# adamnelsonarcher/BB-OCR

Measured on AMD Instinct MI355X. Metric: book-page images/sec end-to-end (detect+recognize) @1280x960, higher is better.
Workload: dtype fp16

## Files before the change

### bb-ocr_amd/csrc/abi.cpp

```cpp
#include "ctx.h"

static hipError_t create_seq_stream(hipStream_t* s) {
    return hipStreamCreateWithFlags(s, hipStreamNonBlocking);
}

extern "C" {

void bbocr_default_params(bbocr_params* p) {
    if (!p) return;
    memset(p, 0, sizeof(*p));
    p->text_threshold = 0.7; p->low_text = 0.4; p->link_threshold = 0.4; p->canvas_size = 2560; p->mag_ratio = 1.0;
    p->slope_ths = 0.1; p->ycenter_ths = 0.5; p->height_ths = 0.5; p->width_ths = 0.5; p->add_margin = 0.1; p->min_size = 20;
    p->contrast_ths = 0.1; p->adjust_contrast = 0.5;
    p->decoder = BBOCR_DECODER_GREEDY; p->beam_width = 5;
}

int bbocr_create(const bbocr_config* cfg, bbocr_ctx** out) {
    bbocr_config_v2 v2{};
    if (cfg) v2.base = *cfg;
    return bbocr_create_v2(&v2, out);
}

int bbocr_create_v2(const bbocr_config_v2* cfg, bbocr_ctx** out) {
    if (!out) return BBOCR_ERR_ARG;
    *out = nullptr;
    bbocr_ctx* c = nullptr;
    try {
        c = new bbocr_ctx();
        c->root = c;
        if (cfg) { c->cfg = cfg->base; c->cfg_beam_wide = cfg->beam_wide; }
        if (c->cfg.precision < BBOCR_PREC_BF16 || c->cfg.precision > BBOCR_PREC_EXACT_REC || c->cfg.call_slots < 0 || c->cfg.call_slots > kMaxSlots ||
            c->cfg.rec_quant < 0 || c->cfg.rec_quant > 1 || (c->cfg.rec_quant == 1 && !rec_split(c)) ||
            c->cfg.rec_classes < 0 || rec_classes(c) < 2 || rec_classes(c) > BBOCR_REC_CLASSES_MAX || c->cfg_beam_wide < 0 || c->cfg_beam_wide > 1 ||
            (c->cfg.rec_quant == 1 && rec_classes(c) != kRecClassesDefault)) {
            delete c;
            return BBOCR_ERR_ARG;
        }
        int ndev = 0;
        if (hipGetDeviceCount(&ndev) != hipSuccess || ndev <= 0 || c->cfg.device < 0 || c->cfg.device >= ndev) {
            delete c;
            return BBOCR_ERR_HIP;
        }
        if (hipSetDevice(c->cfg.device) != hipSuccess || hipStreamCreateWithFlags(&c->stream, hipStreamNonBlocking) != hipSuccess ||
            hipStreamCreateWithFlags(&c->stream2, hipStreamNonBlocking) != hipSuccess ||
            create_seq_stream(&c->seq_stream) != hipSuccess ||
            hipMalloc(&c->zero_page, 256) != hipSuccess || hipMemset(c->zero_page, 0, 256) != hipSuccess) {
            delete c;
            return BBOCR_ERR_HIP;
        }
    } catch (...) {
        delete c;
        return BBOCR_ERR_INTERNAL;
    }
    c->cur = c->stream;
    *out = c;
    return BBOCR_OK;
}

}

bbocr_ctx* slot_create(bbocr_ctx* root) {
    bbocr_ctx* s = new bbocr_ctx();
    s->root = root;
    s->cfg = root->cfg;
    s->cfg_beam_wide = root->cfg_beam_wide;
    s->stream = root->stream;
    hipError_t e = hipStreamCreateWithFlags(&s->stream2, hipStreamNonBlocking);
    if (e == hipSuccess) e = create_seq_stream(&s->seq_stream);
    if (e != hipSuccess) {
        if (s->stream2) (void)hipStreamDestroy(s->stream2);
        delete s;
        fail(BBOCR_ERR_HIP, std::string("call slot: ") + hipGetErrorString(e));
    }
    s->cur = s->stream;
    return s;
}

void slot_destroy(bbocr_ctx* c) {
    if (c->stream2) (void)hipStreamSynchronize(c->stream2);
    if (c->seq_stream) (void)hipStreamSynchronize(c->seq_stream);
    if (c->feat_ev) (void)hipEventDestroy(c->feat_ev);
    for (hipEvent_t e : c->sub_events) (void)hipEventDestroy(e);
    if (c->det_t0) { (void)hipEventDestroy(c->det_t0); (void)hipEventDestroy(c->det_t1); }
    if (c->ccl_t0) { (void)hipEventDestroy(c->ccl_t0); (void)hipEventDestroy(c->ccl_t1); }
    if (c->sync_ev) (void)hipEventDestroy(c->sync_ev);
    if (c->seq_t1) { (void)hipEventDestroy(c->seq_t1); (void)hipEventDestroy(c->seq_t2); }
    for (auto& r : c->prof_recs) { (void)hipEventDestroy(r.e0); (void)hipEventDestroy(r.e1); }
    for (hipEvent_t e : c->prof_pool) (void)hipEventDestroy(e);
    DevBuf* bufs[] = {&c->arena.buf, &c->heat, &c->gray, &c->resized, &c->ccl_label, &c->ccl_stat, &c->ccl_slot, &c->ccl_comps, &c->ccl_rowext,
                      &c->ccl_counters, &c->crop_desc, &c->crop_desc2, &c->crop_scratch, &c->crop_hscratch, &c->crop_wscratch, &c->crop_luts, &c->crop_hist,
                      &c->ctc_idx, &c->ctc_pmax, &c->ctc_out_idx, &c->ctc_out, &c->seq_v, &c->seq_xp, &c->seq_h, &c->seq_lin, &c->seq_logits,
                      &c->seq_tables, &c->pp_gray, &c->pp_a, &c->pp_b, &c->pp_c, &c->pp_tab, &c->ctc_probs, &c->ctc_beam_idx, &c->ctc_beam_len, &c->ctc_cand, &c->ctc_cand_n, &c->ac_work, &c->th_coef, &c->je_scan, &c->je_out, &c->pe_out,
                      &c->pg_rgb, &c->pg_tab, &c->seq_q8, &c->seq_rowp, &c->ctc_mask};
    for (DevBuf* b : bufs) b->release();
    if (c->stream2) (void)hipStreamDestroy(c->stream2);
    if (c->seq_stream) (void)hipStreamDestroy(c->seq_stream);
    if (c->root != c) delete c;
}

namespace {
struct ThreadTimes { const bbocr_ctx* root = nullptr; float ms[8] = {0}; int ctc_route = -1; int ctc_host_seqs = 0; };
thread_local ThreadTimes tl_times;
thread_local std::string tl_err;
struct ThreadMask { const bbocr_ctx* root = nullptr; std::vector<unsigned int> words; };
thread_local ThreadMask tl_mask;
}
const unsigned int* thread_class_mask(const bbocr_ctx* root, int* n_words) {
    const bool mine = tl_mask.root == root && !tl_mask.words.empty();
    *n_words = mine ? (int)tl_mask.words.size() : 0;
    return mine ? tl_mask.words.data() : nullptr;
}
void publish_times(const bbocr_ctx* s) {
    tl_times.root = s->root;
    memcpy(tl_times.ms, s->times, sizeof(tl_times.ms));
    tl_times.ctc_route = s->ctc_last_route;
    tl_times.ctc_host_seqs = s->ctc_host_seqs;
}

extern "C" {

void bbocr_destroy(bbocr_ctx* c) {
    if (!c) return;
    if (tl_mask.root == c) tl_mask = ThreadMask();
    if (tl_times.root == c) tl_times = ThreadTimes();
    (void)hipSetDevice(c->cfg.device);
    if (c->stream) (void)hipStreamSynchronize(c->stream);
    dist_release(c);
    for (bbocr_ctx* s : c->slots) slot_destroy(s);
    c->slots.clear();
    free_weights(c);
    slot_destroy(c);
    if (c->zero_page) (void)hipFree(c->zero_page);
    for (SideLane* l : {&c->upload_lane, &c->jpeg_lane})
        if (l->stream) (void)hipStreamDestroy(l->stream);
    if (c->stream) (void)hipStreamDestroy(c->stream);
    delete c;
}

const char* bbocr_last_error(bbocr_ctx* c) {
    if (!c) return "null context";
    std::lock_guard<std::mutex> lk(c->pool_mu);
    tl_err = c->err;
    return tl_err.c_str();
}

int bbocr_load_weights(bbocr_ctx* ctx, int which, const bbocr_tensor_desc* descs, int n) {
    return guarded(ctx, [&](bbocr_ctx* ctx) {
        if (!descs || n <= 0 || (which != 0 && which != 1)) fail(BBOCR_ERR_ARG, "bad weight descriptor table");
        if (which == 0 ? ctx->craft_loaded : ctx->crnn_loaded)
            fail(BBOCR_ERR_STATE, "this network is already loaded: the packed blocks (and the weight blob layout) are fixed per context -- create a new context");
        TensorMap tm(descs, n);
        if (which == 0) load_craft(ctx, tm);
        else load_crnn(ctx, tm);
    }, true);
}

int bbocr_alloc_weights(bbocr_ctx* ctx, int which) {
    return guarded(ctx, [&](bbocr_ctx* ctx) {
        if (which != 0 && which != 1) fail(BBOCR_ERR_ARG, "which: 0 = detector, 1 = recogniser");
        if (which == 0 ? ctx->craft_loaded : ctx->crnn_loaded)
            fail(BBOCR_ERR_STATE, "this network is already laid out in this context -- create a new context");
        TensorMap tm;
        if (which == 0) load_craft(ctx, tm);
        else load_crnn(ctx, tm);
    }, true);
}

int bbocr_weights_blob_size(bbocr_ctx* ctx, size_t* bytes) {
    return guarded(ctx, [&](bbocr_ctx* ctx) {
        if (!bytes) fail(BBOCR_ERR_ARG, "null pointer");
        *bytes = weights_blob_bytes(ctx);
    }, true);
}

int bbocr_weights_export(bbocr_ctx* ctx, void* dev_blob, size_t bytes) {
    return guarded(ctx, [&](bbocr_ctx* ctx) {
        if (!dev_blob) fail(BBOCR_ERR_ARG, "null device pointer");
        weights_export(ctx, dev_blob, bytes);
    }, true);
}

int bbocr_weights_import(bbocr_ctx* ctx, const void* dev_blob, size_t bytes) {
    return guarded(ctx, [&](bbocr_ctx* ctx) {
        if (!dev_blob) fail(BBOCR_ERR_ARG, "null device pointer");
        weights_import(ctx, dev_blob, bytes);
    }, true);
}

int bbocr_detect_dims(int H, int W, int canvas_size, double mag_ratio, int* H32, int* W32, int* rh, int* rw, double* ratio) {
    if (H <= 0 || W <= 0 || canvas_size <= 0) return BBOCR_ERR_ARG;
    const DetDims d = det_dims(H, W, canvas_size, (double)mag_ratio);
    if (H32) *H32 = d.H32;
    if (W32) *W32 = d.W32;
    if (rh) *rh = d.h;
    if (rw) *rw = d.w;
    if (ratio) *ratio = d.ratio;
    return BBOCR_OK;
}

int bbocr_detect(bbocr_ctx* ctx, const uint8_t* dev_rgb, int B, int H, int W, const bbocr_params* p, float* dev_heat_out) {
    return guarded(ctx, [&](bbocr_ctx* ctx) {
        bbocr_params pp;
        bbocr_default_params(&pp);
        if (p) pp = *p;
        if (!dev_rgb || !dev_heat_out) fail(BBOCR_ERR_ARG, "null device pointer");
        memset(ctx->times, 0, sizeof(ctx->times));
        auto t0 = clk::now();
        detect_impl(ctx, dev_rgb, B, H, W, pp, dev_heat_out);
        slot_sync(ctx, ctx->stream);
        prof_collect(ctx);
        ctx->times[0] = ctx->times[7] = (float)ms_since(t0);
    });
}

int bbocr_boxes(bbocr_ctx* ctx, const float* dev_heat, int B, int h, int w, double ratio, const bbocr_params* p, bbocr_boxlist** out) {
    return guarded(ctx, [&](bbocr_ctx* ctx) {
        bbocr_params pp;
        bbocr_default_params(&pp);
        if (p) pp = *p;
        if (!dev_heat || !out) fail(BBOCR_ERR_ARG, "null pointer");
        memset(ctx->times, 0, sizeof(ctx->times));
        auto t0 = clk::now();
        HostBoxes hb;
        boxes_impl(ctx, dev_heat, B, h, w, ratio, pp, hb, ctx->stream);
        *out = export_boxes(hb);
        ctx->times[7] = (float)ms_since(t0);
    });
}

int bbocr_recognize(bbocr_ctx* ctx, const uint8_t* dev_gray, int B, int H, int W, const bbocr_boxlist* boxes, const bbocr_params* p,
                    bbocr_result** out) {
    return guarded(ctx, [&](bbocr_ctx* ctx) {
        bbocr_params pp;
        bbocr_default_params(&pp);
        if (p) pp = *p;
        if (!dev_gray || !boxes || !out || boxes->n_images != B) fail(BBOCR_ERR_ARG, "bad recognise arguments");
        memset(ctx->times, 0, sizeof(ctx->times));
        auto t0 = clk::now();
        HostBoxes hb;
        import_boxes(boxes, hb);
        std::vector<BoxJob> jobs;
        std::vector<int> off;
        recognize_impl(ctx, GrayPages{dev_gray, H, W}, B, hb, pp, jobs, off);
        prof_collect(ctx);
        *out = export_result(B, jobs, off);
        ctx->times[7] = (float)ms_since(t0);
    });
}

int bbocr_readtext_batch(bbocr_ctx* ctx, const uint8_t* dev_rgb, const uint8_t* dev_gray, int B, int H, int W, const bbocr_params* p,
                         bbocr_result** out) {
    return guarded(ctx, [&](bbocr_ctx* ctx) {
        bbocr_params pp;
        bbocr_default_params(&pp);
        if (p) pp = *p;
        if (!dev_rgb || !out) fail(BBOCR_ERR_ARG, "null pointer");
        memset(ctx->times, 0, sizeof(ctx->times));
        auto t_all = clk::now();
        const DetDims d = det_dims(H, W, pp.canvas_size, pp.mag_ratio);
        ctx->heat.ensure((size_t)B * d.h * d.w * 2 * sizeof(float));
        if (!dev_gray) {
            ctx->gray.ensure((size_t)B * H * W);
            HIPCHK(launch_gray(dev_rgb, (uint8_t*)ctx->gray.p, (size_t)B * H * W, ctx->stream));
            dev_gray = (const uint8_t*)ctx->gray.p;
        }
        std::vector<std::pair<int, int>> subs;
        if (!ctx->det_t0) { HIPCHK(hipEventCreate(&ctx->det_t0)); HIPCHK(hipEventCreate(&ctx->det_t1)); }
        HIPCHK(hipEventRecord(ctx->det_t0, ctx->stream));
        detect_impl(ctx, dev_rgb, B, H, W, pp, (float*)ctx->heat.p, [&](int b0, int nb) {
            if (subs.size() >= ctx->sub_events.size()) {
                hipEvent_t e;
                HIPCHK(hipEventCreateWithFlags(&e, hipEventDisableTiming));
                ctx->sub_events.push_back(e);
            }
            HIPCHK(hipEventRecord(ctx->sub_events[subs.size()], ctx->stream));
            subs.push_back({b0, nb});
        });
        HIPCHK(hipEventRecord(ctx->det_t1, ctx->stream));
        HostBoxes hb;
        hb.polys.resize(B); hb.hori.resize(B); hb.freeb.resize(B);
        RecEarly early;
        for (size_t k = 0; k < subs.size(); ++k) {
            const int b0 = subs[k].first, nb = subs[k].second;
            HIPCHK(hipStreamWaitEvent(ctx->stream2, ctx->sub_events[k], 0));
            HostBoxes part;
            boxes_impl(ctx, (const float*)ctx->heat.p + (size_t)b0 * d.h * d.w * 2, nb, d.h, d.w, d.ratio, pp, part, ctx->stream2);
            for (int i = 0; i < nb; ++i) {
                hb.polys[b0 + i] = std::move(part.polys[i]);
                hb.hori[b0 + i] = std::move(part.hori[i]);
                hb.freeb[b0 + i] = std::move(part.freeb[i]);
            }
            if (subs.size() >= 2 && k + 2 == subs.size() && pp.rotation_info[0] == 0 && ctx->crnn_loaded)
                rec_early_begin(ctx, GrayPages{dev_gray, H, W}, b0 + nb, B, hb, pp, early);
        }
        HIPCHK(hipEventSynchronize(ctx->det_t1));
        float det_ms = 0.f;
        HIPCHK(hipEventElapsedTime(&det_ms, ctx->det_t0, ctx->det_t1));
        ctx->times[0] = det_ms;
        std::vector<BoxJob> jobs;
        std::vector<int> off;
        recognize_impl(ctx, GrayPages{dev_gray, H, W}, B, hb, pp, jobs, off, &early);
        prof_collect(ctx);
        *out = export_result(B, jobs, off);
        ctx->times[7] = (float)ms_since(t_all);
    });
}

void bbocr_preproc_defaults(bbocr_preproc_params* p, int legacy) {
    if (!p) return;
    memset(p, 0, sizeof(*p));
    p->scale = 1.5; p->unsharp_radius = 1.0; p->unsharp_threshold = 3;
    if (legacy) { p->blur_sigma = 5.0; p->contrast = 1.3; p->brightness = 0.0; p->clahe_clip = 2.0; p->unsharp_percent = 20; }
    else        { p->blur_sigma = 3.0; p->contrast = 1.9; p->brightness = 1.2; p->clahe_clip = 2.5; p->unsharp_percent = 30; }
}

int bbocr_preprocess_chain(bbocr_ctx* ctx, const uint8_t* dev_bgr, int H, int W, const bbocr_preproc_params* p, uint8_t* dev_out, int* out_h,
                           int* out_w) {
    return guarded(ctx, [&](bbocr_ctx* ctx) {
        bbocr_preproc_params q;
        bbocr_preproc_defaults(&q, 0);
        if (p) q = *p;
        if (H <= 0 || W <= 0) fail(BBOCR_ERR_ARG, "bad image shape");
        if (q.scale < 0 || q.blur_sigma < 0 || q.contrast < 0 || q.brightness < 0 || q.clahe_clip < 0 || q.unsharp_radius < 0 || q.unsharp_percent < 0)
            fail(BBOCR_ERR_ARG, "negative pre-processing parameter");
        const int dh = q.scale > 0 ? (int)(H * q.scale) : H, dw = q.scale > 0 ? (int)(W * q.scale) : W;
        if (out_h) *out_h = dh;
        if (out_w) *out_w = dw;
        if (!dev_out) return;
        if (!dev_bgr) fail(BBOCR_ERR_ARG, "null device pointer");
        if (dh <= 0 || dw <= 0) fail(BBOCR_ERR_ARG, "image collapses to zero size");
        if (q.clahe_clip > 0 && (dh < 16 || dw < 16)) fail(BBOCR_ERR_ARG, "image too small for the 8x8 CLAHE tile grid");
        preprocess_chain_impl(ctx, dev_bgr, H, W, q, dev_out, dh, dw);
    });
}

int bbocr_preprocess_book_cover(bbocr_ctx* ctx, const uint8_t* dev_bgr, int H, int W, uint8_t* dev_out, int* out_h, int* out_w) {
    bbocr_preproc_params q;
    bbocr_preproc_defaults(&q, 0);
    return bbocr_preprocess_chain(ctx, dev_bgr, H, W, &q, dev_out, out_h, out_w);
}

void bbocr_free_boxlist(bbocr_boxlist* b) {
    if (!b) return;
    free(b->poly_off); free(b->polys); free(b->hori_off); free(b->hori); free(b->free_off); free(b->free_q);
    free(b);
}

void bbocr_free_result(bbocr_result* r) {
    if (!r) return;
    free(r->box_off); free(r->quads); free(r->is_free); free(r->text_off); free(r->text_idx); free(r->conf);
    free(r);
}

int bbocr_set_class_mask(bbocr_ctx* ctx, const uint32_t* words, int n_words) {
    return status_of(ctx, [&] {
        if (!rec_wide(ctx)) fail(BBOCR_ERR_ARG, "bbocr_set_class_mask is for contexts of more than 128 classes; bbocr_params::ignore_mask rules here");
        const int C = rec_classes(ctx), max_words = (C + 31) / 32;
        if (n_words < 0 || n_words > max_words || (n_words > 0 && !words)) fail(BBOCR_ERR_ARG, "class mask: 0 .. " + std::to_string(max_words) + " words");
        if (n_words > 0 && (words[0] & 1u)) fail(BBOCR_ERR_ARG, "the CTC blank (class 0) cannot be ignored");
        if (n_words == max_words && (C & 31) && (words[n_words - 1] >> (C & 31))) fail(BBOCR_ERR_ARG, "class mask: a bit behind the last class is set");
        tl_mask.root = n_words > 0 ? ctx : nullptr;
        tl_mask.words.assign(words, words + n_words);
    });
}

int bbocr_last_ctc_route(bbocr_ctx* ctx, int* route) {
    if (!ctx || !route) return BBOCR_ERR_ARG;
    *route = tl_times.root == ctx ? tl_times.ctc_route : -1;
    return BBOCR_OK;
}

int bbocr_last_ctc_host_sequences(bbocr_ctx* ctx, int* n) {
    if (!ctx || !n) return BBOCR_ERR_ARG;
    *n = tl_times.root == ctx ? tl_times.ctc_host_seqs : 0;
    return BBOCR_OK;
}

int bbocr_set_profiling(bbocr_ctx* ctx, int on) {
    return guarded(ctx, [&](bbocr_ctx* c) {
        c->profiling = on < 0 ? 0 : (on > 2 ? 2 : on);
        std::lock_guard<std::mutex> lk(c->pool_mu);
        for (int g = 0; g < 2; ++g) { c->prof_ms[g] = 0; c->prof_flops[g] = 0; c->prof_launches[g] = 0; }
    }, true);
}

int bbocr_conv_profile(bbocr_ctx* ctx, int group, double* ms, double* flops, long long* launches) {
    if (!ctx || group < 0 || group > 1) return BBOCR_ERR_ARG;
    std::lock_guard<std::mutex> lk(ctx->pool_mu);
    if (ms) *ms = ctx->prof_ms[group];
    if (flops) *flops = ctx->prof_flops[group];
    if (launches) *launches = ctx->prof_launches[group];
    return BBOCR_OK;
}

int bbocr_stage_times(bbocr_ctx* ctx, float* ms, int n) {
    if (!ctx || !ms || n <= 0) return BBOCR_ERR_ARG;
    for (int i = 0; i < n && i < 8; ++i) ms[i] = tl_times.root == ctx ? tl_times.ms[i] : 0.f;
    return BBOCR_OK;
}


}
```

### bb-ocr_amd/csrc/ccl.hip

```cpp
#include "common.h"
#include "kernels.h"

__device__ __forceinline__ int ccl_find(const int* __restrict__ label, int x) {
    int p = __hip_atomic_load(label + x, __ATOMIC_RELAXED, __HIP_MEMORY_SCOPE_AGENT);
    while (p != x) {
        x = p;
        p = __hip_atomic_load(label + x, __ATOMIC_RELAXED, __HIP_MEMORY_SCOPE_AGENT);
    }
    return x;
}

__device__ __forceinline__ void ccl_union(int* label, int a, int b) {
    for (;;) {
        a = ccl_find(label, a);
        b = ccl_find(label, b);
        if (a == b) return;
        if (a > b) { const int t = a; a = b; b = t; }
        const int old = atomicMin(label + b, a);
        if (old == b) return;
        b = old;
    }
}

__global__ void __launch_bounds__(256) ccl_init_kernel(const float* __restrict__ heat, size_t total, int w, float low_text, float link_thr,
                                                       int* __restrict__ label, int* __restrict__ stat, int* __restrict__ slot) {
    const int lane = threadIdx.x & 63;
    const size_t nround = (total + (size_t)gridDim.x * 256 - 1) / ((size_t)gridDim.x * 256);
    for (size_t it = 0; it < nround; ++it) {
        const size_t i = (it * gridDim.x + blockIdx.x) * 256 + threadIdx.x;
        bool fg = false;
        int x = 0;
        if (i < total) {
            const float2 v = *(const float2*)(heat + i * 2);
            fg = (v.x > low_text) || (v.y > link_thr);
            x = (int)(i % w);
        }
        const unsigned long long fgm = __ballot(fg);
        const bool start = fg && (lane == 0 || x == 0 || !((fgm >> (lane - 1)) & 1ULL));
        const unsigned long long sm = __ballot(start);
        if (i < total) {
            int lab = -1;
            if (fg) {
                const unsigned long long below = sm & ((lane == 63) ? ~0ULL : ((1ULL << (lane + 1)) - 1ULL));
                lab = (int)i - (lane - (63 - __clzll((long long)below)));
            }
            label[i] = lab;
            slot[i] = -1;
            int* st = stat + i * 6;
            st[0] = 0x7fffffff; st[1] = -1; st[2] = 0x7fffffff; st[3] = -1; st[4] = 0; st[5] = 0;
        }
    }
}

__global__ void __launch_bounds__(256) ccl_merge_kernel(size_t total, int h, int w, int* label) {
    for (size_t i = (size_t)blockIdx.x * 256 + threadIdx.x; i < total; i += (size_t)gridDim.x * 256) {
        if (label[i] < 0) continue;
        const int x = (int)(i % w);
        const int y = (int)((i / w) % h);
        const bool left = x > 0 && label[i - 1] >= 0;
        if (left && (i & 63) == 0) ccl_union(label, (int)i, (int)i - 1);
        if (y > 0 && label[i - w] >= 0 && !(left && label[i - w - 1] >= 0)) ccl_union(label, (int)i, (int)i - w);
    }
}

__global__ void __launch_bounds__(256) ccl_stats_kernel(const float* __restrict__ heat, size_t total, int h, int w, int* label,
                                                        int* __restrict__ stat) {
    const int lane = threadIdx.x & 63;
    const size_t nround = (total + (size_t)gridDim.x * 256 - 1) / ((size_t)gridDim.x * 256);
    for (size_t it = 0; it < nround; ++it) {
        const size_t i = (it * gridDim.x + blockIdx.x) * 256 + threadIdx.x;
        int r = -1, x = 0, y = 0;
        float t = 0.f;
        if (i < total && label[i] >= 0) {
            r = ccl_find(label, (int)i);
            label[i] = r;
            x = (int)(i % w);
            y = (int)((i / w) % h);
            t = fmaxf(heat[i * 2], 0.f);
        }
        const int rp = __shfl_up(r, 1);
        const bool head = r >= 0 && (lane == 0 || rp != r || x == 0);
        const unsigned long long hm = __ballot(head || r < 0);
        if (r >= 0) {
            const unsigned long long below = hm & ((lane == 63) ? ~0ULL : ((1ULL << (lane + 1)) - 1ULL));
            const int first = 63 - __clzll((long long)below);
            const unsigned long long above = (lane == 63) ? 0ULL : (hm >> (lane + 1));
            const int len_after = above ? (__ffsll((long long)above) - 1) : (63 - lane);
            float m = t;
#pragma unroll
            for (int o = 1; o < 64; o <<= 1) {
                const float mo = __shfl_down(m, o);
                if (o <= len_after) m = fmaxf(m, mo);
            }
            if (head) {
                int* st = stat + (size_t)r * 6;
                atomicMin(st + 0, x);
                atomicMax(st + 1, x + len_after);
                atomicMin(st + 2, y);
                atomicMax(st + 3, y);
                atomicAdd(st + 4, len_after + 1);
                if (m > 0.f) atomicMax(st + 5, __float_as_int(m));
            }
            (void)first;
        }
    }
}

__global__ void __launch_bounds__(256) ccl_accept_kernel(size_t total, int hw, double text_thr, const int* __restrict__ label,
                                                         const int* __restrict__ stat, int* __restrict__ slot, CclOut* comps,
                                                         int* rowext, int* counters, int cap_comps, int cap_rows) {
    for (size_t i = (size_t)blockIdx.x * 256 + threadIdx.x; i < total; i += (size_t)gridDim.x * 256) {
        if (label[i] != (int)i) continue;
        const int* st = stat + i * 6;
        const int area = st[4];
        if (area < 10) continue;
        if ((double)__int_as_float(st[5]) < text_thr) continue;
        const int img = (int)(i / hw);
        const int hh = st[3] - st[2] + 1;
        const int idx = atomicAdd(counters + 0, 1);
        const int off = atomicAdd(counters + 1, hh);
        if (idx >= cap_comps || off + hh > cap_rows) { atomicOr(counters + 2, 1); continue; }
        CclOut c;
        c.root = (int)(i - (size_t)img * hw);
        c.left = st[0]; c.top = st[2]; c.right = st[1]; c.bottom = st[3]; c.area = area; c.row_off = off; c.img = img;
        comps[idx] = c;
        slot[i] = idx;
        int* re = rowext + (size_t)off * 2;
        for (int k = 0; k < hh; ++k) { re[2 * k] = 0x7fffffff; re[2 * k + 1] = -1; }
    }
}

__global__ void __launch_bounds__(256) ccl_rowext_kernel(const float* __restrict__ heat, size_t total, int h, int w, float low_text,
                                                         const int* __restrict__ label, const int* __restrict__ slot,
                                                         const CclOut* __restrict__ comps, int* rowext, int cap_comps, int cap_rows) {
    const int lane = threadIdx.x & 63;
    const size_t nround = (total + (size_t)gridDim.x * 256 - 1) / ((size_t)gridDim.x * 256);
    for (size_t it = 0; it < nround; ++it) {
        const size_t i = (it * gridDim.x + blockIdx.x) * 256 + threadIdx.x;
        int r = -1, x = 0;
        if (i < total) {
            r = label[i];
            if (r >= 0 && !(heat[i * 2] > low_text)) r = -1;
            x = (int)(i % w);
        }
        const int rp = __shfl_up(r, 1);
        const bool head = r >= 0 && (lane == 0 || rp != r || x == 0);
        const unsigned long long hm = __ballot(head || r < 0);
        if (head) {
            const int s = slot[r];
            if (s >= 0) {
                const unsigned long long above = (lane == 63) ? 0ULL : (hm >> (lane + 1));
                const int len_after = above ? (__ffsll((long long)above) - 1) : (63 - lane);
                const CclOut c = comps[s];
                const int y = (int)((i / w) % h);
                int* re = rowext + ((size_t)c.row_off + (y - c.top)) * 2;
                atomicMin(re, x);
                atomicMax(re + 1, x + len_after);
            }
        }
    }
}

hipError_t launch_ccl(const float* heat, int N, int h, int w, float low_text, float link_thr, double text_thr, int* label, int* stat,
                      int* slot, CclOut* comps, int* rowext, int* counters, int cap_comps, int cap_rows, hipStream_t s) {
    const size_t total = (size_t)N * h * w;
    if (total == 0) return hipSuccess;
    if (total > 0x7fffffffULL) return hipErrorInvalidValue;
    const int grid = (int)((total + 255) / 256 < 16384 ? (total + 255) / 256 : 16384);
    hipError_t e = hipMemsetAsync(counters, 0, sizeof(int) * 4, s);
    if (e != hipSuccess) return e;
    hipLaunchKernelGGL(ccl_init_kernel, dim3(grid), dim3(256), 0, s, heat, total, w, low_text, link_thr, label, stat, slot);
    hipLaunchKernelGGL(ccl_merge_kernel, dim3(grid), dim3(256), 0, s, total, h, w, label);
    hipLaunchKernelGGL(ccl_stats_kernel, dim3(grid), dim3(256), 0, s, heat, total, h, w, label, stat);
    hipLaunchKernelGGL(ccl_accept_kernel, dim3(grid), dim3(256), 0, s, total, h * w, text_thr, label, stat, slot, comps, rowext, counters,
                       cap_comps, cap_rows);
    hipLaunchKernelGGL(ccl_rowext_kernel, dim3(grid), dim3(256), 0, s, heat, total, h, w, low_text, label, slot, comps, rowext, cap_comps,
                       cap_rows);
    return hipGetLastError();
}
```

### bb-ocr_amd/csrc/crnn_misc.hip

```cpp
#include "common.h"
#include "kernels.h"

template <bool PAGES>
__global__ void __launch_bounds__(256) crop_warp_kernel(const uint8_t* __restrict__ gray, int H, int W, const CropDesc* __restrict__ descs,
                                                        int first, uint8_t* __restrict__ wscratch, const CropPage* __restrict__ pages) {
    const CropDesc d = descs[first + blockIdx.y];
    if (!d.warp) return;
    const uint8_t* src;
    size_t pitch;
    if constexpr (PAGES) {
        const CropPage pg = pages[d.img];
        src = gray + pg.off; H = pg.H; W = pg.W; pitch = (size_t)pg.pitch;
    } else {
        src = gray + (size_t)d.img * H * W; pitch = (size_t)W;
    }
    uint8_t* dst = wscratch + d.warp_off;
    const int total = d.sw * d.sh;
    for (int i = blockIdx.x * 256 + threadIdx.x; i < total; i += gridDim.x * 256) {
        const int x = i % d.sw, y = i / d.sw;
        const double X0 = d.Minv[0] * (double)x + (d.Minv[1] * (double)y + d.Minv[2]);
        const double Y0 = d.Minv[3] * (double)x + (d.Minv[4] * (double)y + d.Minv[5]);
        const double W0 = d.Minv[6] * (double)x + (d.Minv[7] * (double)y + d.Minv[8]);
        const double Wi = W0 != 0.0 ? 32.0 / W0 : 0.0;
        double fX = X0 * Wi, fY = Y0 * Wi;
        fX = fX < -2147483648.0 ? -2147483648.0 : (fX > 2147483647.0 ? 2147483647.0 : fX);
        fY = fY < -2147483648.0 ? -2147483648.0 : (fY > 2147483647.0 ? 2147483647.0 : fY);
        const long long X = (long long)rint(fX), Y = (long long)rint(fY);
        long long sxl = X >> 5, syl = Y >> 5;
        sxl = sxl < -32768 ? -32768 : (sxl > 32767 ? 32767 : sxl);
        syl = syl < -32768 ? -32768 : (syl > 32767 ? 32767 : syl);
        const int sx = (int)sxl, sy = (int)syl;
        const int ax = (int)(X & 31), ay = (int)(Y & 31);
        auto tap = [&](int yy, int xx) -> int {
            return (yy >= 0 && yy < H && xx >= 0 && xx < W) ? (int)src[(size_t)yy * pitch + xx] : 0;
        };
        const int acc = tap(sy, sx) * ((32 - ax) * (32 - ay) * 32) + tap(sy, sx + 1) * (ax * (32 - ay) * 32) +
                        tap(sy + 1, sx) * ((32 - ax) * ay * 32) + tap(sy + 1, sx + 1) * (ax * ay * 32);
        int v = (acc + (1 << 14)) >> 15;
        dst[i] = (uint8_t)(v < 0 ? 0 : (v > 255 ? 255 : v));
    }
}

__device__ __forceinline__ void cv_lin_coef_d(int d, int ssize, double scale, int& s0, int& s1, int& a0, int& a1) {
    float fx = (float)(((double)d + 0.5) * scale - 0.5);
    int sx = (int)floorf(fx);
    fx -= (float)sx;
    if (sx < 0) { fx = 0.f; sx = 0; }
    if (sx >= ssize - 1) { fx = 0.f; sx = ssize - 1; }
    a0 = __float2int_rn((1.f - fx) * 2048.f);
    a1 = __float2int_rn(fx * 2048.f);
    s0 = sx;
    s1 = sx + 1 < ssize ? sx + 1 : ssize - 1;
}

template <bool PAGES>
__global__ void __launch_bounds__(256) crop_resize_kernel(const uint8_t* __restrict__ gray, int H, int W, const CropDesc* __restrict__ descs,
                                                          int first, const uint8_t* __restrict__ wscratch, uint8_t* __restrict__ scratch,
                                                          const CropPage* __restrict__ pages) {
    const CropDesc d = descs[first + blockIdx.y];
    const uint8_t* src;
    size_t stride;
    if (d.warp) { src = wscratch + d.warp_off; stride = (size_t)d.sw; }
    else if constexpr (PAGES) {
        const CropPage pg = pages[d.img];
        src = gray + pg.off + (size_t)d.sy0 * (size_t)pg.pitch + d.sx0; stride = (size_t)pg.pitch;
    }
    else { src = gray + (size_t)d.img * H * W + (size_t)d.sy0 * W + d.sx0; stride = (size_t)W; }
    uint8_t* dst = scratch + d.a_off;
    const int sw = d.sw, sh = d.sh, dw = (d.rot & 1) ? d.rh : d.rw, dh = (d.rot & 1) ? d.rw : d.rh;
    const bool same = (dw == sw && dh == sh), area2 = (sw == 2 * dw && sh == 2 * dh);
    const double scale_x = 1.0 / ((double)dw / (double)sw), scale_y = 1.0 / ((double)dh / (double)sh);
    const int total = dw * dh;
    for (int i = blockIdx.x * 256 + threadIdx.x; i < total; i += gridDim.x * 256) {
        const int dx = i % dw, dy = i / dw;
        int v;
        if (same) {
            v = src[(size_t)dy * stride + dx];
        } else if (area2) {
            v = (src[(size_t)(2 * dy) * stride + 2 * dx] + src[(size_t)(2 * dy) * stride + 2 * dx + 1] +
                 src[(size_t)(2 * dy + 1) * stride + 2 * dx] + src[(size_t)(2 * dy + 1) * stride + 2 * dx + 1] + 2) >> 2;
        } else {
            int x0, x1, a0, a1, y0, y1, b0, b1;
            cv_lin_coef_d(dx, sw, scale_x, x0, x1, a0, a1);
            cv_lin_coef_d(dy, sh, scale_y, y0, y1, b0, b1);
            const int r0 = src[(size_t)y0 * stride + x0] * a0 + src[(size_t)y0 * stride + x1] * a1;
            const int r1 = src[(size_t)y1 * stride + x0] * a0 + src[(size_t)y1 * stride + x1] * a1;
            v = (((b0 * (r0 >> 4)) >> 16) + ((b1 * (r1 >> 4)) >> 16) + 2) >> 2;
            v = v < 0 ? 0 : (v > 255 ? 255 : v);
        }
        int o = i;
        if (d.rot == 1) o = (dw - 1 - dx) * dh + dy;
        else if (d.rot == 2) o = (dh - 1 - dy) * dw + (dw - 1 - dx);
        else if (d.rot == 3) o = dx * dh + (dh - 1 - dy);
        dst[o] = (uint8_t)v;
    }
}

__global__ void __launch_bounds__(256) crop_hist_kernel(const uint8_t* __restrict__ scratch, const CropDesc* __restrict__ descs, int first,
                                                        unsigned int* __restrict__ hist) {
    __shared__ unsigned int h[256];
    const CropDesc d = descs[first + blockIdx.x];
    h[threadIdx.x] = 0;
    __syncthreads();
    const uint8_t* p = scratch + d.a_off;
    const int total = d.rw * d.rh;
    for (int i = threadIdx.x; i < total; i += 256) atomicAdd(&h[p[i]], 1u);
    __syncthreads();
    hist[(size_t)blockIdx.x * 256 + threadIdx.x] = h[threadIdx.x];
}

#define PIL_PREC 22
__device__ __forceinline__ double pil_bicubic(double x) {
    const double a = -0.5;
    if (x < 0.0) x = -x;
    if (x < 1.0) return ((a + 2.0) * x - (a + 3.0)) * x * x + 1;
    if (x < 2.0) return (((x - 5) * x + 8) * x - 4) * a;
    return 0.0;
}
struct PilWin { int x0, n; double center, ss, ww; };
__device__ PilWin pil_window(int in_size, int out_size, int xx) {
    double scale = (double)in_size / (double)out_size, filterscale = scale;
    if (filterscale < 1.0) filterscale = 1.0;
    const double support = 2.0 * filterscale;
    PilWin w;
    w.center = ((double)xx + 0.5) * scale;
    w.ss = 1.0 / filterscale;
    int x0 = (int)(w.center - support + 0.5);
    if (x0 < 0) x0 = 0;
    int x1 = (int)(w.center + support + 0.5);
    if (x1 > in_size) x1 = in_size;
    w.x0 = x0;
    w.n = x1 - x0;
    w.ww = 0.0;
    for (int x = 0; x < w.n; ++x) w.ww += pil_bicubic(((double)(x + x0) - w.center + 0.5) * w.ss);
    return w;
}
__device__ __forceinline__ int pil_tap(const PilWin& w, int x) {
    double k = pil_bicubic(((double)(x + w.x0) - w.center + 0.5) * w.ss);
    if (w.ww != 0.0) k = k / w.ww;
    return k < 0 ? (int)(-0.5 + k * (double)(1 << PIL_PREC)) : (int)(0.5 + k * (double)(1 << PIL_PREC));
}
__device__ __forceinline__ int pil_clip8(long long v) {
    const long long r = v >> PIL_PREC;
    return r < 0 ? 0 : (r > 255 ? 255 : (int)r);
}

__global__ void __launch_bounds__(256) crop_pil_h_kernel(const CropDesc* __restrict__ descs, int first, const uint8_t* __restrict__ scratch,
                                                         const uint8_t* __restrict__ luts, uint8_t* __restrict__ hscratch) {
    const CropDesc d = descs[first + blockIdx.y];
    if (d.fw == d.rw && d.rh == 64) return;
    const uint8_t* src = scratch + d.a_off;
    const uint8_t* lut = d.lut_off >= 0 ? luts + d.lut_off : nullptr;
    uint8_t* dst = hscratch + d.a_off;
    const int total = d.rh * d.fw;
    for (int i = blockIdx.x * 256 + threadIdx.x; i < total; i += gridDim.x * 256) {
        const int xx = i % d.fw, y = i / d.fw;
        int v;
        if (d.fw == d.rw) {
            v = src[(size_t)y * d.rw + xx];
            if (lut) v = lut[v];
        } else {
            const PilWin win = pil_window(d.rw, d.fw, xx);
            long long acc = 1LL << (PIL_PREC - 1);
            for (int k = 0; k < win.n; ++k) {
                int p = src[(size_t)y * d.rw + win.x0 + k];
                if (lut) p = lut[p];
                acc += (long long)p * pil_tap(win, k);
            }
            v = pil_clip8(acc);
        }
        dst[i] = (uint8_t)v;
    }
}

template <int MODE>
__global__ void __launch_bounds__(256) crop_final_kernel(const CropDesc* __restrict__ descs, int first, const uint8_t* __restrict__ scratch,
                                                         const uint8_t* __restrict__ hscratch, const uint8_t* __restrict__ luts,
                                                         uint16_t* __restrict__ out, int row_stride, long long slot_stride, int gap) {
    const CropDesc d = descs[first + blockIdx.y];
    const bool tall = !(d.fw == d.rw && d.rh == 64);
    const uint8_t* src = (tall ? hscratch : scratch) + d.a_off;
    const uint8_t* lut = (!tall && d.lut_off >= 0) ? luts + d.lut_off : nullptr;
    uint16_t* dst = out + (size_t)d.slot * (size_t)slot_stride;
    const int imgW = d.imgW;
    const int t = blockIdx.x * 256 + threadIdx.x;
    const int y = t >> 6, x0 = t & 63;
    if (y >= 64) return;
    const bool vert = tall && d.rh != 64;
    PilWin win;
    if (vert) win = pil_window(d.rh, 64, y);
    auto sample = [&](int xs) {
        int v;
        if (!tall) {
            v = src[(size_t)y * d.rw + xs];
            if (lut) v = lut[v];
        } else if (!vert) {
            v = src[(size_t)y * d.fw + xs];
        } else {
            long long acc = 1LL << (PIL_PREC - 1);
            for (int k = 0; k < win.n; ++k) acc += (long long)src[(size_t)(win.x0 + k) * d.fw + xs] * pil_tap(win, k);
            v = pil_clip8(acc);
        }
        if constexpr (MODE == REC_SPLIT) return (unsigned short)(v + 1);
        else return El<MODE == REC_F16 ? 1 : 0>::from_f32(((float)v / 255.0f - 0.5f) / 0.5f);
    };
    uint16_t* drow = dst + (size_t)y * row_stride;
    for (int x = imgW + x0; x < imgW + gap; x += 64) drow[x] = 0;
    int x = x0;
    for (; x < d.fw; x += 64) drow[x] = sample(x);
    if (x < imgW) {
        const uint16_t edge = sample(d.fw - 1);
        for (; x < imgW; x += 64) drow[x] = edge;
    }
}

hipError_t launch_crops(const uint8_t* gray, int H, int W, const CropDesc* descs_dev, int first, int count, int imgW, int any_warp,
                        int any_tall, uint8_t* wscratch, uint8_t* scratch, uint8_t* hscratch, const uint8_t* luts, uint16_t* out_bucket,
                        int stage_mask, hipStream_t s, int wide_row_stride, int gap, int mode, const CropPage* pages) {
    if (count <= 0) return hipSuccess;
    if ((stage_mask & 1) && pages) {
        if (any_warp) hipLaunchKernelGGL(crop_warp_kernel<true>, dim3(16, count), dim3(256), 0, s, gray, 0, 0, descs_dev, first, wscratch, pages);
        hipLaunchKernelGGL(crop_resize_kernel<true>, dim3(16, count), dim3(256), 0, s, gray, 0, 0, descs_dev, first, wscratch, scratch, pages);
    } else if (stage_mask & 1) {
        if (any_warp) hipLaunchKernelGGL(crop_warp_kernel<false>, dim3(16, count), dim3(256), 0, s, gray, H, W, descs_dev, first, wscratch, pages);
        hipLaunchKernelGGL(crop_resize_kernel<false>, dim3(16, count), dim3(256), 0, s, gray, H, W, descs_dev, first, wscratch, scratch, pages);
    }
    if (stage_mask & 2) {
        if (any_tall) hipLaunchKernelGGL(crop_pil_h_kernel, dim3(8, count), dim3(256), 0, s, descs_dev, first, scratch, luts, hscratch);
        const int rs = wide_row_stride > 0 ? wide_row_stride : imgW;
        const long long ss = wide_row_stride > 0 ? 1LL : (long long)64 * imgW;
        const int gp = wide_row_stride > 0 ? gap : 0;
        if (mode == REC_SPLIT)
            hipLaunchKernelGGL(crop_final_kernel<REC_SPLIT>, dim3(16, count), dim3(256), 0, s, descs_dev, first, scratch, hscratch, luts, out_bucket, rs, ss, gp);
        else if (mode == REC_F16)
            hipLaunchKernelGGL(crop_final_kernel<REC_F16>, dim3(16, count), dim3(256), 0, s, descs_dev, first, scratch, hscratch, luts, out_bucket, rs, ss, gp);
        else
            hipLaunchKernelGGL(crop_final_kernel<REC_BF16>, dim3(16, count), dim3(256), 0, s, descs_dev, first, scratch, hscratch, luts, out_bucket, rs, ss, gp);
    }
    return hipGetLastError();
}

hipError_t launch_crop_hist(const uint8_t* scratch, const CropDesc* descs_dev, int first, int count, unsigned int* hist, hipStream_t s) {
    if (count <= 0) return hipSuccess;
    hipLaunchKernelGGL(crop_hist_kernel, dim3(count), dim3(256), 0, s, scratch, descs_dev, first, hist);
    return hipGetLastError();
}

template <int MODE>
__global__ void __launch_bounds__(256) crnn_conv0_kernel(const uint16_t* __restrict__ in, const float* __restrict__ w,
                                                         const float* __restrict__ b, uint16_t* __restrict__ out, int n, int W) {
    const int OW = W / 2, OH = 32;
    const size_t total = (size_t)n * OH * OW;
    for (size_t i = (size_t)blockIdx.x * 256 + threadIdx.x; i < total; i += (size_t)gridDim.x * 256) {
        const int ox = (int)(i % OW);
        const size_t r = i / OW;
        const int oy = (int)(r % OH);
        const int img = (int)(r / OH);
        const uint16_t* p = in + (size_t)img * 64 * W;
        float v[4][4];
#pragma unroll
        for (int dy = 0; dy < 4; ++dy)
#pragma unroll
            for (int dx = 0; dx < 4; ++dx) {
                const int iy = 2 * oy - 1 + dy, ix = 2 * ox - 1 + dx;
                float x = 0.f;
                if (iy >= 0 && iy < 64 && ix >= 0 && ix < W) {
                    const unsigned short q = p[(size_t)iy * W + ix];
                    if constexpr (MODE == REC_SPLIT) x = q ? ((float)(q - 1) / 255.0f - 0.5f) / 0.5f : 0.f;
                    else x = El<MODE == REC_F16 ? 1 : 0>::to_f32(q);
                }
                v[dy][dx] = x;
            }
        uint16_t* op = out + i * (MODE == REC_SPLIT ? 64 : 32);
#pragma unroll 1
        for (int c8 = 0; c8 < 32; c8 += 8) {
            u32x4 o, ol;
#pragma unroll
            for (int c2 = 0; c2 < 4; ++c2) {
                const int c = c8 + c2 * 2;
                const f32x2_t bias = {b[c], b[c + 1]};
                f32x2_t best = {0.f, 0.f};
#pragma unroll
                for (int py = 0; py < 2; ++py)
#pragma unroll
                    for (int px = 0; px < 2; ++px) {
                        f32x2_t a = bias;
#pragma unroll
                        for (int ky = 0; ky < 3; ++ky)
#pragma unroll
                            for (int kx = 0; kx < 3; ++kx) {
                                const f32x2_t wv = *(const f32x2_t*)(w + (ky * 3 + kx) * 32 + c);
                                const float x = v[py + ky][px + kx];
                                a = __builtin_elementwise_fma(wv, (f32x2_t){x, x}, a);
                            }
                        best = __builtin_elementwise_max(best, a);
                    }
                if constexpr (MODE == REC_SPLIT) {
                    const float h0 = El<1>::to_f32(El<1>::from_f32(best[0])), h1 = El<1>::to_f32(El<1>::from_f32(best[1]));
                    o[c2] = El<1>::pack2(h0, h1);
                    ol[c2] = El<1>::pack2((best[0] - h0) * SPLIT_LO_SCALE, (best[1] - h1) * SPLIT_LO_SCALE);
                } else {
                    o[c2] = El<MODE == REC_F16 ? 1 : 0>::pack2(best[0], best[1]);
                }
            }
            *(u32x4*)(op + c8) = o;
            if constexpr (MODE == REC_SPLIT) *(u32x4*)(op + 32 + c8) = ol;
        }
    }
}

void pack_crnn_conv0_mfma(const float* w_tap_major, uint16_t* out, int el) {
    size_t o = 0;
    for (int j = 0; j < 2; ++j)
        for (int l = 0; l < 64; ++l) {
            const int m = l & 15, kg = l >> 4;
            const int cout = 8 * (m >> 2) + 4 * j + (m & 3);
            for (int t = 0; t < 8; ++t) {
                const float v = w_tap_major[t * 32 + cout];
                const float hi = el_to_f32_host(el, f32_to_el_host(el, v));
                const float lo = el_to_f32_host(el, f32_to_el_host(el, v - hi));
                const float lo2 = el_to_f32_host(el, f32_to_el_host(el, (v - hi) - lo));
                out[o++] = f32_to_el_host(el, kg == 0 ? hi : (kg == 1 ? lo : (kg == 2 ? lo2 : 0.f)));
            }
        }
}

template <int EL>
__global__ void __launch_bounds__(256) crnn_conv0_mfma_kernel(const uint16_t* __restrict__ in, const uint16_t* __restrict__ afrag, const float* __restrict__ w,
                                                              const float* __restrict__ b, uint16_t* __restrict__ out, int W) {
    constexpr int TW = 64, PITCH = TW + 16, ROWS = 66;
    __shared__ __attribute__((aligned(16))) uint16_t tile[ROWS * PITCH];
    typedef typename El<EL>::v8 v8;
    const int tid = threadIdx.x, lane = tid & 63, wave = tid >> 6;
    const int g = lane >> 4, n = lane & 15;
    const int x0 = blockIdx.x * TW, img = blockIdx.y;
    const int OW = W >> 1;
    const uint16_t* src = in + (size_t)img * 64 * W;
    for (int idx = tid; idx < ROWS * (PITCH / 4); idx += 256) {
        const int row = idx / (PITCH / 4), ch = idx - row * (PITCH / 4);
        const int iy = row - 1, ix = x0 - 8 + ch * 4;
        u32x2 v = {0u, 0u};
        if (iy >= 0 && iy < 64 && ix >= 0 && ix + 4 <= W) v = *(const u32x2*)(src + (size_t)iy * W + ix);
        *(u32x2*)(tile + row * PITCH + ch * 4) = v;
    }
    const v8 a0 = *(const v8*)(afrag + (size_t)lane * 8), a1 = *(const v8*)(afrag + (size_t)(64 + lane) * 8);
    float w8[8], bi[8];
#pragma unroll
    for (int i = 0; i < 8; ++i) {
        w8[i] = w[8 * 32 + 8 * g + i];
        bi[i] = b[8 * g + i];
    }
    __syncthreads();
    auto frag = [&](int y, int cf, f32x4& d0, f32x4& d1) {
        const uint16_t* p = tile + (y + 1) * PITCH + 8 + cf * 16 + n;
        u32x4 bq;
#pragma unroll
        for (int i = 0; i < 4; ++i) {
            const int t0 = 2 * i, t1 = 2 * i + 1;
            const unsigned int lo = p[(t0 / 3 - 1) * PITCH + (t0 % 3 - 1)], hi = p[(t1 / 3 - 1) * PITCH + (t1 % 3 - 1)];
            bq[i] = lo | (hi << 16);
        }
        const float x8 = El<EL>::to_f32(p[PITCH + 1]);
        d0 = El<EL>::mfma(a0, __builtin_bit_cast(v8, bq), (f32x4){bi[0], bi[1], bi[2], bi[3]});
        d1 = El<EL>::mfma(a1, __builtin_bit_cast(v8, bq), (f32x4){bi[4], bi[5], bi[6], bi[7]});
#pragma unroll
        for (int r = 0; r < 4; ++r) {
            d0[r] = fmaf(w8[r], x8, d0[r]);
            d1[r] = fmaf(w8[4 + r], x8, d1[r]);
        }
    };
#pragma unroll 1
    for (int rp = 0; rp < 8; ++rp) {
        const int y = 2 * (wave * 8 + rp);
#pragma unroll
        for (int cf = 0; cf < 4; ++cf) {
            f32x4 u0, u1, l0, l1;
            frag(y, cf, u0, u1);
            frag(y + 1, cf, l0, l1);
            float m[8];
#pragma unroll
            for (int r = 0; r < 4; ++r) {
                m[r] = __builtin_fmaxf(__builtin_fmaxf(u0[r], l0[r]), 0.f);
                m[4 + r] = __builtin_fmaxf(__builtin_fmaxf(u1[r], l1[r]), 0.f);
            }
#pragma unroll
            for (int i = 0; i < 8; ++i)
                m[i] = fmaxf(m[i], __int_as_float(__builtin_amdgcn_update_dpp(0, __float_as_int(m[i]), 0xB1 , 0xF, 0xF, true)));
            const int px = (x0 + cf * 16 + n) >> 1;
            if (!(n & 1) && px < OW) {
                const u32x4 o = {El<EL>::pack2(m[0], m[1]), El<EL>::pack2(m[2], m[3]), El<EL>::pack2(m[4], m[5]), El<EL>::pack2(m[6], m[7])};
                *(u32x4*)(out + (((size_t)img * 32 + (y >> 1)) * OW + px) * 32 + 8 * g) = o;
            }
        }
    }
}

hipError_t launch_crnn_conv0(const uint16_t* in, const float* w, const float* b, uint16_t* out, int n, int W, int mode, hipStream_t s,
                             const uint16_t* afrag) {
    const size_t total = (size_t)n * 32 * (W / 2);
    if (total == 0) return hipSuccess;
    if (afrag && mode != REC_SPLIT && (W & 3) == 0 && n <= 65535) {
        const dim3 grid((W + 63) / 64, n);
        if (mode == REC_F16) hipLaunchKernelGGL(crnn_conv0_mfma_kernel<1>, grid, dim3(256), 0, s, in, afrag, w, b, out, W);
        else hipLaunchKernelGGL(crnn_conv0_mfma_kernel<0>, grid, dim3(256), 0, s, in, afrag, w, b, out, W);
        return hipGetLastError();
    }
    const int grid = (int)((total + 255) / 256 < 16384 ? (total + 255) / 256 : 16384);
    if (mode == REC_SPLIT) hipLaunchKernelGGL(crnn_conv0_kernel<REC_SPLIT>, dim3(grid), dim3(256), 0, s, in, w, b, out, n, W);
    else if (mode == REC_F16) hipLaunchKernelGGL(crnn_conv0_kernel<REC_F16>, dim3(grid), dim3(256), 0, s, in, w, b, out, n, W);
    else hipLaunchKernelGGL(crnn_conv0_kernel<REC_BF16>, dim3(grid), dim3(256), 0, s, in, w, b, out, n, W);
    return hipGetLastError();
}

template <int MODE>
__device__ __forceinline__ void rowmean3_8(const uint16_t* p0, const uint16_t* p1, const uint16_t* p2, uint16_t* o, int lo_off) {
    typedef El<MODE == REC_BF16 ? 0 : 1> E;
    const u32x4 a = *(const u32x4*)(p0), bq = *(const u32x4*)(p1), c = *(const u32x4*)(p2);
    u32x4 oh, ol;
    if constexpr (MODE == REC_SPLIT) {
        const u32x4 al = *(const u32x4*)(p0 + lo_off), bl = *(const u32x4*)(p1 + lo_off), cl = *(const u32x4*)(p2 + lo_off);
        const float inv = 1.0f / SPLIT_LO_SCALE;
#pragma unroll
        for (int j = 0; j < 4; ++j) {
            const f32x2_t m = ((E::unpack2(a[j]) + E::unpack2(al[j]) * inv) + (E::unpack2(bq[j]) + E::unpack2(bl[j]) * inv) +
                               (E::unpack2(c[j]) + E::unpack2(cl[j]) * inv)) / 3.0f;
            const f32x2_t h = E::unpack2(E::pack2(m[0], m[1]));
            oh[j] = E::pack2(h[0], h[1]);
            ol[j] = E::pack2((m[0] - h[0]) * SPLIT_LO_SCALE, (m[1] - h[1]) * SPLIT_LO_SCALE);
        }
        *(u32x4*)(o) = oh;
        *(u32x4*)(o + lo_off) = ol;
    } else {
#pragma unroll
        for (int j = 0; j < 4; ++j) {
            const f32x2_t m = (E::unpack2(a[j]) + E::unpack2(bq[j]) + E::unpack2(c[j])) / 3.0f;
            oh[j] = E::pack2(m[0], m[1]);
        }
        *(u32x4*)(o) = oh;
    }
}

__global__ void __launch_bounds__(256) crnn_zero_gaps_kernel(uint16_t* __restrict__ t, const CropDesc* __restrict__ descs, int first, int H, int Wl,
                                                             int C8, int shift, int gapw) {
    const CropDesc d = descs[first + blockIdx.x];
    const int x0 = (d.slot + d.imgW) >> shift;
    const int total = H * gapw * C8;
    for (int i = threadIdx.x; i < total; i += 256) {
        const int c8 = i % C8, r = i / C8;
        const int gx = r % gapw, y = r / gapw;
        if (x0 + gx < Wl) *(u32x4*)(t + ((size_t)y * Wl + x0 + gx) * C8 * 8 + (size_t)c8 * 8) = (u32x4){0u, 0u, 0u, 0u};
    }
}
hipError_t launch_crnn_zero_gaps(uint16_t* t, const CropDesc* descs_dev, int first, int count, int H, int Wl, int C, int shift, hipStream_t s) {
    if (count <= 0) return hipSuccess;
    hipLaunchKernelGGL(crnn_zero_gaps_kernel, dim3(count), dim3(256), 0, s, t, descs_dev, first, H, Wl, C / 8, shift, 4 >> shift);
    return hipGetLastError();
}

template <int MODE>
__global__ void __launch_bounds__(256) rowmean3_gather_kernel(const uint16_t* __restrict__ in, int Wc, int C8, const CropDesc* __restrict__ descs,
                                                              int first, uint16_t* __restrict__ out) {
    constexpr int M = MODE == REC_SPLIT ? 2 : 1;
    const CropDesc d = descs[first + blockIdx.y];
    const int T = d.imgW / 4 - 1, xs = d.slot >> 2;
    const size_t plane = (size_t)Wc * C8 * 8 * M;
    const int total = T * C8;
    for (int i = blockIdx.x * 256 + threadIdx.x; i < total; i += gridDim.x * 256) {
        const int t = i / C8, c8 = i - t * C8;
        const uint16_t* p = in + ((size_t)(xs + t) * C8 * M + c8) * 8;
        rowmean3_8<MODE>(p, p + plane, p + 2 * plane, out + ((size_t)(d.pad_ + t) * C8 * M + c8) * 8, C8 * 8);
    }
}
hipError_t launch_rowmean3_gather(const uint16_t* in, int Wc, int C, const CropDesc* descs_dev, int first, int count, uint16_t* out, int mode,
                                  hipStream_t s) {
    if (count <= 0) return hipSuccess;
    if (mode == REC_SPLIT) hipLaunchKernelGGL(rowmean3_gather_kernel<REC_SPLIT>, dim3(8, count), dim3(256), 0, s, in, Wc, C / 8, descs_dev, first, out);
    else if (mode == REC_F16) hipLaunchKernelGGL(rowmean3_gather_kernel<REC_F16>, dim3(8, count), dim3(256), 0, s, in, Wc, C / 8, descs_dev, first, out);
    else hipLaunchKernelGGL(rowmean3_gather_kernel<REC_BF16>, dim3(8, count), dim3(256), 0, s, in, Wc, C / 8, descs_dev, first, out);
    return hipGetLastError();
}
```

### bb-ocr_amd/csrc/ctx.h

```cpp
#pragma once
#include "../../include/bbocr.h"

#include <algorithm>
#include <atomic>
#include <chrono>
#include <condition_variable>
#include <cmath>
#include <cstring>
#include <functional>
#include <map>
#include <memory>
#include <mutex>
#include <string>
#include <thread>
#include <unordered_map>
#include <vector>

#include "boxpost.h"
#include "hostpool.h"
#include "common.h"
#include "kernels.h"


using clk = std::chrono::steady_clock;
static inline double ms_since(clk::time_point t0) { return std::chrono::duration<double, std::milli>(clk::now() - t0).count(); }
static inline size_t align_up(size_t v, size_t a) { return (v + a - 1) / a * a; }
static inline int cdiv(int a, int b) { return (a + b - 1) / b; }

struct StatusError {
    int code;
    std::string msg;
};
[[noreturn]] inline void fail(int code, const std::string& m) { throw StatusError{code, m}; }
#define HIPCHK(expr)                                                                                   \
    do {                                                                                               \
        hipError_t _e = (expr);                                                                        \
        if (_e != hipSuccess) fail(BBOCR_ERR_HIP, std::string(#expr) + ": " + hipGetErrorString(_e));  \
    } while (0)

struct DevBuf {
    void* p = nullptr;
    size_t cap = 0;
    DevBuf() = default;
    DevBuf(const DevBuf&) = delete;
    DevBuf& operator=(const DevBuf&) = delete;
    ~DevBuf() { release(); }
    void ensure(size_t n) {
        if (n <= cap) return;
        if (p) (void)hipFree(p);
        p = nullptr;
        cap = 0;
        HIPCHK(hipMalloc(&p, n));
        cap = n;
    }
    void ensure_keep(size_t n, size_t used) {
        if (n <= cap) return;
        void* q = nullptr;
        HIPCHK(hipDeviceSynchronize());
        HIPCHK(hipMalloc(&q, n));
        if (p && used) HIPCHK(hipMemcpy(q, p, std::min(used, cap), hipMemcpyDeviceToDevice));
        if (p) (void)hipFree(p);
        p = q;
        cap = n;
    }
    void release() {
        if (p) (void)hipFree(p);
        p = nullptr;
        cap = 0;
    }
};

struct PinBuf {
    void* p = nullptr;
    size_t cap = 0;
    PinBuf() = default;
    PinBuf(const PinBuf&) = delete;
    PinBuf& operator=(const PinBuf&) = delete;
    ~PinBuf() { if (p) (void)hipHostFree(p); }
    void ensure(size_t n) {
        if (n <= cap) return;
        if (p) { HIPCHK(hipDeviceSynchronize()); (void)hipHostFree(p); }
        p = nullptr;
        cap = 0;
        HIPCHK(hipHostMalloc(&p, n, hipHostMallocDefault));
        cap = n;
    }
};

struct Arena {
    DevBuf buf;
    size_t off = 0;
    bool dry = true;
    void begin(bool d) { off = 0; dry = d; }
    template <typename T> T* alloc(size_t count) {
        off = align_up(off, 256);
        T* r = dry ? nullptr : (T*)((char*)buf.p + off);
        off += count * sizeof(T);
        return r;
    }
};

struct Carve {
    size_t off = 0;
    size_t add(size_t bytes) { const size_t o = off; off = align_up(off + bytes, 256); return o; }
    template <typename T> static T* at(void* base, size_t o) { return (T*)((char*)base + o); }
};

struct Act {
    uint16_t* p;
    int N, H, W, C;
};

struct DevPage {
    const void* p;
    int H, W;
    long long pitch;
    int layout;
};
constexpr unsigned page_set(int layout) { return 1u << layout; }
constexpr unsigned PAGE_ANY = page_set(PAGE_YCC3 + 1) - 1;
inline void check_page(const DevPage& g, unsigned allowed = PAGE_ANY) {
    if (!g.p) fail(BBOCR_ERR_ARG, "null device pointer");
    if (g.H < 1 || g.W < 1) fail(BBOCR_ERR_ARG, "bad image shape");
    if ((long long)g.H * g.W >= (1LL << 30)) fail(BBOCR_ERR_ARG, "image too large");
    if (g.layout < PAGE_GRAY || g.layout > PAGE_YCC3 || !(allowed & page_set(g.layout))) fail(BBOCR_ERR_ARG, "layout must be one of the BBOCR_PAGE_* taken here");
    if (g.pitch < (long long)g.W * page_px_bytes(g.layout)) fail(BBOCR_ERR_ARG, "row pitch smaller than a row");
}

struct SideLane {
    std::mutex mu;
    hipStream_t stream = nullptr;
};



struct WeightView {
    bool craft_loaded = false;
    uint16_t* c11_wf = nullptr;
    float* c11_b = nullptr;
    float* c11_w32 = nullptr;
    float* cls6_w32 = nullptr;
    ConvPlan conv1_2, conv2_1, conv2_2, conv3_1, conv3_2, conv3_3, conv4_1, conv4_2, conv4_3, conv5_1, conv5_2, fc6, fc7;
    ConvPlan up1a, up1b, up2b, up3b, up4b, cls0, cls2, cls4;
    ConvPlan up2y, up2s, up3y, up3s, up4y, up4s;
    float* cls_tail = nullptr;
    uint16_t* cls_tail_frag = nullptr;
    uint16_t* up4y_post = nullptr;
    bool crnn_loaded = false;
    float* r0_wb = nullptr;
    uint16_t* r0_afrag = nullptr;
    ConvPlan r1, r2, r3, r4, r5, r6, xproj[2], lin[2], pred;
    uint16_t* pred_wide = nullptr;
    float* pred_wide_b = nullptr;
    uint16_t* whh[2] = {nullptr, nullptr};
    float whh_scale[2] = {1.f, 1.f};
    struct Q8Layer { int8_t* w = nullptr; float* scale = nullptr; float* bias = nullptr; };
    Q8Layer q_ih[2], q_hh[2], q_lin[2], q_pred;
    void* zero_page = nullptr;
};

struct bbocr_ctx : WeightView {
    bbocr_config cfg{};
    int cfg_beam_wide = 0;
    bbocr_ctx* root = nullptr;
    std::vector<bbocr_ctx*> slots;
    std::mutex pool_mu;
    std::condition_variable pool_cv;
    std::mutex enq_mu;
    ConvRoute op_conv_route{};
    bool slot_busy = false;
    hipStream_t stream = nullptr;
    DevBuf pp_gray, pp_a, pp_b, pp_c, pp_tab;
    DevBuf ac_work;
    DevBuf th_coef;
    int th_coef_key[6] = {0, 0, 0, 0, 0, 0};
    int th_coef_ks[2] = {0, 0};
    int th_coef_rows[2] = {0, 0};
    DevBuf je_scan, je_out;
    DevBuf pe_out;
    DevBuf pp_cubic;
    int pp_cubic_key[4] = {0, 0, 0, 0};
    unsigned long long pp_cubic_K[2] = {0, 0};
    unsigned int ignore_mask[4] = {0, 0, 0, 0};
    int beam_width = 0;
    std::vector<unsigned int> class_mask;
    DevBuf ctc_mask;
    int ctc_host_seqs = 0;
    int ctc_last_route = -1;
    hipStream_t cur = nullptr;
    SideLane upload_lane;
    SideLane jpeg_lane;
    PinBuf jd_pin;
    DevBuf jd_in, jd_work, jd_coef, jd_stage;
    DevBuf jd_page;
    long long jd_count[4] = {0, 0, 0, 0};
    hipStream_t seq_stream = nullptr;
    hipEvent_t feat_ev = nullptr;
    hipStream_t stream2 = nullptr;
    std::vector<hipEvent_t> sub_events;
    hipEvent_t ccl_t0 = nullptr, ccl_t1 = nullptr;
    hipEvent_t det_t0 = nullptr, det_t1 = nullptr;
    hipEvent_t sync_ev = nullptr;
    hipEvent_t seq_t1 = nullptr, seq_t2 = nullptr;
    std::string err;
    float times[8] = {0};

    struct ProfRec { hipEvent_t e0, e1; double flops; int group; };
    int profiling = 0;
    int prof_group = 0;
    std::vector<ProfRec> prof_recs;
    std::vector<hipEvent_t> prof_pool;
    double prof_ms[2] = {0, 0}, prof_flops[2] = {0, 0};
    long long prof_launches[2] = {0, 0};

    void* dist_comm = nullptr;
    int dist_rank = 0, dist_world = 0;
    std::unique_ptr<HostPool> pool;
    std::vector<void*> owned;
    std::vector<size_t> owned_bytes;

    Arena arena;
    DevBuf heat, gray, resized;
    DevBuf pg_rgb, pg_tab;
    PinBuf pg_pin;
    DevBuf ccl_label, ccl_stat, ccl_slot, ccl_comps, ccl_rowext, ccl_counters;
    DevBuf crop_desc, crop_scratch, crop_hscratch, crop_wscratch, crop_luts, crop_hist;
    DevBuf ctc_idx, ctc_pmax, ctc_out_idx, ctc_out, ctc_probs, ctc_beam_idx, ctc_beam_len, ctc_cand, ctc_cand_n, crop_desc2;
    PinBuf desc_pin, desc_pin2;
    PinBuf ctc_pin;
    DevBuf seq_v, seq_xp, seq_h, seq_lin, seq_logits, seq_tables;
    DevBuf seq_q8, seq_rowp;
};

inline int det_el(const bbocr_ctx* c) { return (c->cfg.precision == BBOCR_PREC_FP16 || c->cfg.precision == BBOCR_PREC_EXACT || c->cfg.precision == BBOCR_PREC_EXACT_REC) ? 1 : 0; }
inline int rec_el(const bbocr_ctx* c) { return c->cfg.precision != BBOCR_PREC_BF16 ? 1 : 0; }
inline bool rec_split(const bbocr_ctx* c) { return c->cfg.precision == BBOCR_PREC_EXACT || c->cfg.precision == BBOCR_PREC_EXACT_REC; }
inline bool rec_quant(const bbocr_ctx* c) { return c->cfg.rec_quant == 1; }
constexpr int kRecClassesDefault = 97;
inline int rec_classes(const bbocr_ctx* c) { return c->cfg.rec_classes > 0 ? c->cfg.rec_classes : kRecClassesDefault; }
inline int rec_cs(const bbocr_ctx* c) { return (rec_classes(c) + 15) / 16 * 16; }
inline bool rec_wide(const bbocr_ctx* c) { return rec_classes(c) > 128; }
inline bool rec_beam_wide(const bbocr_ctx* c) { return c->cfg_beam_wide == 1 && rec_wide(c); }
inline bool det_split(const bbocr_ctx* c) { return c->cfg.precision == BBOCR_PREC_EXACT; }

struct TensorMap {
    std::unordered_map<std::string, const bbocr_tensor_desc*> m;
    bool zeros = false;
    std::vector<float> zero_buf;
    TensorMap() : zeros(true), zero_buf((size_t)5 << 20, 0.f) {}
    TensorMap(const bbocr_tensor_desc* d, int n) {
        for (int i = 0; i < n; ++i) {
            std::string k = d[i].name ? d[i].name : "";
            if (k.rfind("module.", 0) == 0) k = k.substr(7);
            m[k] = &d[i];
        }
    }
    const float* get(const std::string& name, size_t numel, bool required = true) const {
        if (zeros) {
            if (zero_buf.size() < numel) fail(BBOCR_ERR_INTERNAL, "allocation-only load: tensor '" + name + "' larger than the zero buffer");
            return zero_buf.data();
        }
        auto it = m.find(name);
        if (it == m.end()) {
            if (required) fail(BBOCR_ERR_WEIGHTS, "missing tensor '" + name + "'");
            return nullptr;
        }
        size_t n = 1;
        for (int i = 0; i < it->second->ndim; ++i) n *= (size_t)it->second->shape[i];
        if (n != numel || !it->second->data)
            fail(BBOCR_ERR_WEIGHTS, "tensor '" + name + "' has " + std::to_string(n) + " elements, expected " + std::to_string(numel));
        return it->second->data;
    }
};

struct RgbSource { const uint8_t* rgb; int Himg, Wimg; };

struct DetDims {
    int H32, W32, h, w, th, tw;
    double ratio;
};

struct DetPlan {
    int H, W;
    DetDims d;
    std::vector<int> passes;
    size_t arena_bytes, resized_bytes;
};

struct GrayPages {
    const uint8_t* gray;
    int H, W;
    const CropPage* tab = nullptr;
    const CropPage* tab_dev = nullptr;
    int h(int b) const { return tab ? tab[b].H : H; }
    int w(int b) const { return tab ? tab[b].W : W; }
};

struct HostBoxes {
    std::vector<std::vector<std::array<int, 8>>> polys;
    std::vector<std::vector<std::array<int, 4>>> hori;
    std::vector<std::vector<std::array<double, 8>>> freeb;
};

struct BoxJob {
    int img;
    bool is_free;
    double quad[8];
    CropDesc d;
    std::vector<int> text;
    double conf = 0.0;
};

struct RecChunk {
    int imgW, T, first, n;
    size_t row0;
};

struct RecPart {
    std::vector<CropDesc> descs;
    std::vector<int> order;
    std::vector<RecChunk> chunks;
    size_t rows = 0, cols = 0;
    bool any_warp = false, any_tall = false;
};

struct RecRun {
    std::vector<int> tiles, seqs, seq_k;
    size_t rows = 0;
    int n_results = 0;
};

struct RecEarly {
    bool active = false;
    int pages = 0;
    std::vector<BoxJob> jobs;
    std::vector<int> box_off;
    size_t a_total = 0, w_total = 0;
    RecPart part;
};

constexpr int REC_GAP = 4;
constexpr int REC_STAGES = 8;

template <typename T> inline T* upload(bbocr_ctx* c, const std::vector<T>& v) {
    void* d = nullptr;
    HIPCHK(hipMalloc(&d, v.size() * sizeof(T)));
    c->owned.push_back(d);
    c->owned_bytes.push_back(v.size() * sizeof(T));
    HIPCHK(hipMemcpy(d, v.data(), v.size() * sizeof(T), hipMemcpyHostToDevice));
    return (T*)d;
}

ConvPlan make_plan(int Cin, int Cout, int KH, int KW, int pad, int dil, int el = 0, int bn = 0);
void upload_plan(bbocr_ctx* c, ConvPlan& p, const std::vector<float>& w, const std::vector<float>& b);
void free_weights(bbocr_ctx* c);
size_t weights_blob_bytes(const bbocr_ctx* c);
void weights_export(bbocr_ctx* c, void* dev_dst, size_t bytes);
void weights_import(bbocr_ctx* c, const void* dev_src, size_t bytes);
void load_craft(bbocr_ctx* c, const TensorMap& tm);
void load_crnn(bbocr_ctx* c, const TensorMap& tm);
ConvArgs conv_args(const ConvPlan& p, const Act& a0, const Act* a1 = nullptr, const Act* addup = nullptr);
hipError_t launch_conv_profiled(bbocr_ctx* c, const ConvPlan& p, ConvArgs a, bool may_decline = false);
void run_conv(bbocr_ctx* c, const ConvPlan& p, const Act& a0, bool relu0, const Act* a1, bool relu1, bool relu_out, void* out, int out_cs, int cout_store, bool out_f32, const Act* addup = nullptr);
hipError_t launch_seq_proj_profiled(bbocr_ctx* c, const ConvPlan& p, const uint16_t* x, size_t rows_pad, uint16_t* out);
void prof_collect(bbocr_ctx* c);
Act conv_act(bbocr_ctx* c, const ConvPlan& p, const Act& a0, bool relu0, const Act* a1, bool relu1, bool relu_out, int store);
Act conv_pool_act(bbocr_ctx* c, const ConvPlan& p, const Act& a0, bool relu0, bool relu_out, int store, int mode, bool pool_relu, Act* full, const RgbSource* rgb = nullptr);
Act pool_act(bbocr_ctx* c, const Act& a, int kh, int kw, int sh, int sw, int ph, int pw, bool relu_in);
void craft_up_stage(bbocr_ctx* c, const ConvPlan& py, const ConvPlan& ps, const Act& y, const Act& skip, uint16_t* z, uint16_t* out);
bool craft_up3b_post(bbocr_ctx* c, const Act& u3a, uint16_t* u3b, uint16_t* z);
bool craft_up4(bbocr_ctx* c, const Act& s1, const uint16_t* z, uint16_t* u4b);
void craft_cls_tail(bbocr_ctx* c, const Act& c2, float* heat);
struct ExactConvRow {
    const char* name;
    ConvPlan bbocr_ctx::* plan;
    bool relu_out;
    int store;
    int pool_mode;
    bool pool_relu;
    bool keep_full;
};
int craft_exact_rows();
const ExactConvRow& craft_exact_row(int row);
Act craft_exact_conv(bbocr_ctx* c, int row, const Act& in, Act* full = nullptr);
Act craft_exact_conv1_1(bbocr_ctx* c, const uint8_t* rgb, int nb, int Himg, int Wimg, int H32, int W32);
Act craft_exact_relu(bbocr_ctx* c, const Act& a);
Act craft_exact_upcat(bbocr_ctx* c, const Act& y, const Act& skip);
Act craft_exact_pool5(bbocr_ctx* c, const Act& s4);
void craft_exact_cls_tail(bbocr_ctx* c, const Act& c3, float* heat);
DetDims det_dims(int H, int W, int canvas, double mag);
void detect_impl(bbocr_ctx* c, const uint8_t* rgb, int B, int H, int W, const bbocr_params& p, float* heat, const std::function<void(int, int)>& after_sub = nullptr);
DetPlan det_plan(bbocr_ctx* c, int B, int H, int W, const bbocr_params& p, bool overlapped);
void det_size(bbocr_ctx* c, size_t arena_bytes, size_t resized_bytes);
void det_run(bbocr_ctx* c, const DetPlan& s, const uint8_t* rgb, float* heat, const std::function<void(int, int)>& after_sub = nullptr);
int ccl_cap_comps(int B, int h, int w);
void ccl_size(bbocr_ctx* c, size_t npx, int cap_comps);
void boxes_impl(bbocr_ctx* c, const float* heat, int B, int h, int w, double ratio, const bbocr_params& p, HostBoxes& hb, hipStream_t st);
bbocr_boxlist* export_boxes(const HostBoxes& hb);
void import_boxes(const bbocr_boxlist* bl, HostBoxes& hb);
bool plan_horizontal(const std::array<int, 4>& box, int img, int H, int W, BoxJob& j);
bool plan_free(const std::array<double, 8>& fq, int img, BoxJob& j);
int rec_mode(const bbocr_ctx* c);
void crop_refit_fw(CropDesc& d);
void rec_layout_scratch(std::vector<BoxJob>& jobs, size_t first, size_t& a_total, size_t& w_total);
bool contrast_lut(const unsigned int* hist, size_t npx, double target, uint8_t* lut);
std::vector<int> crop_contrast_luts(bbocr_ctx* c, const CropDesc* descs_dev, std::vector<CropDesc>& descs, double target, std::vector<uint8_t>& luts);
void rec_launch_crops(bbocr_ctx* c, const GrayPages& g, const RecPart& part, const CropDesc* dd, uint16_t* wide, int stage);
void rec_plan_part(const std::vector<BoxJob>& jobs, const std::vector<int>& sel, int res0, size_t row_base, RecPart& part);
const CropDesc* rec_upload_descs(bbocr_ctx* c, const RecPart& part, DevBuf& desc_buf);
uint16_t* rec_wide_image(bbocr_ctx* c, const RecPart& part);
void crnn_features_wide(bbocr_ctx* c, const RecPart& part, const CropDesc* descs, const uint16_t* wide);
Act crnn_stage_shape(const bbocr_ctx* c, const RecPart& part, int stage);
Act crnn_features_stages(bbocr_ctx* c, const RecPart& part, const CropDesc* descs, Act a, int first, int last);
void rec_add_tables(RecRun& run, const RecPart& part, int tile_seqs);
void crnn_sequence(bbocr_ctx* c, size_t rows, size_t rows_pad, const int* tiles_dev, int ntiles, const int* seqs_dev, int nseq, float* logits);
void crnn_seq_xproj(bbocr_ctx* c, int l, const uint16_t* x, size_t rows_pad, void* xp);
void crnn_seq_xproj_conv(bbocr_ctx* c, int l, const uint16_t* x, size_t rows_pad, void* xp);
void crnn_seq_lin(bbocr_ctx* c, int l, const uint16_t* h, size_t rows_pad, uint16_t* out);
void crnn_seq_pred(bbocr_ctx* c, const uint16_t* x, size_t rows_pad, float* logits);
void rec_seq_tiles(const bbocr_ctx* c, RecRun& run);
enum { CTC_GREEDY = 0, CTC_BEAM_HOST = 1, CTC_BEAM_DEVICE = 2, CTC_GREEDY_FUSED = 3, CTC_BEAM_DEVICE_WIDE = 4 };
int ctc_route(int beam_width, int C, const int* seqs, int nseq, bool fused_ok = false, bool beam_wide = false);
int ctc_beam_wide_fallback(bbocr_ctx* c, hipStream_t s, const float* probs_dev, const int* seqs, int nseq, int C, int cs, int beam_width, const int* blen,
                           std::vector<std::vector<int>>& texts);
const unsigned int* thread_class_mask(const bbocr_ctx* root, int* n_words);
void ctc_size(bbocr_ctx* c, size_t rows, int nseq, int cs, int route);
double ctc_decode(const CtcOut& o, const int* idx, int n, std::vector<int>& text);
void rec_early_begin(bbocr_ctx* c, const GrayPages& g, int pages, int B, const HostBoxes& hb, const bbocr_params& p, RecEarly& e);
void recognize_impl(bbocr_ctx* c, const GrayPages& g, int B, const HostBoxes& hb, const bbocr_params& p, std::vector<BoxJob>& jobs, std::vector<int>& box_off, RecEarly* early = nullptr);
bbocr_result* export_result(int B, const std::vector<BoxJob>& jobs, const std::vector<int>& box_off);
void pp_resize(bbocr_ctx* c, const uint8_t* src, int H, int W, uint8_t* dst, int dh, int dw, bool src_bgr = false);
void pp_gauss(bbocr_ctx* c, const uint8_t* src, int H, int W, uint8_t* dst, double sigma);
const uint8_t* pp_fold_lut(bbocr_ctx* c, size_t n, double contrast, double brightness);
void pp_clahe(bbocr_ctx* c, const uint8_t* src, int H, int W, const uint8_t* d_lut, uint8_t* dst, double clip_limit);
void pp_unsharp(bbocr_ctx* c, const uint8_t* src, int H, int W, uint8_t* dst, uint8_t* tmp1, uint8_t* tmp2, float radius, int percent, int threshold);
void preprocess_chain_impl(bbocr_ctx* c, const uint8_t* bgr, int H, int W, const bbocr_preproc_params& q, uint8_t* out, int dh, int dw);
void gaussian_taps_fixed(int n, double sigma, int* k);

inline HostPool& host_pool(bbocr_ctx* c) {
    if (!c->pool) {
        const int want = c->cfg.host_threads > 0 ? c->cfg.host_threads : std::min(16, host_cpu_share());
        c->pool.reset(new HostPool(std::max(1, std::min(want, 64)) - 1));
    }
    return *c->pool;
}

inline bool other_call_in_flight(bbocr_ctx* c) {
    bbocr_ctx* root = c->root;
    std::lock_guard<std::mutex> lk(root->pool_mu);
    if (root != c && root->slot_busy) return true;
    for (bbocr_ctx* s : root->slots)
        if (s != c && s->slot_busy) return true;
    return false;
}

struct EnqLock {
    std::unique_lock<std::mutex> lk;
    explicit EnqLock(bbocr_ctx* c) : lk(c->root->enq_mu) {}
};
constexpr int kMaxSlots = 2;
bbocr_ctx* slot_create(bbocr_ctx* root);
void slot_destroy(bbocr_ctx* s);
void publish_times(const bbocr_ctx* s);
void dist_release(bbocr_ctx* root);

inline void slot_sync(bbocr_ctx* c, hipStream_t st) {
    if (!c->sync_ev) HIPCHK(hipEventCreateWithFlags(&c->sync_ev, hipEventDisableTiming));
    HIPCHK(hipEventRecord(c->sync_ev, st));
    HIPCHK(hipEventSynchronize(c->sync_ev));
}

inline void prof_release(bbocr_ctx* c, const bbocr_ctx::ProfRec& r) { c->prof_pool.push_back(r.e0); c->prof_pool.push_back(r.e1); }

inline void guarded_drain(bbocr_ctx* ctx) {
    if (ctx->stream) (void)hipStreamSynchronize(ctx->stream);
    if (ctx->stream2) (void)hipStreamSynchronize(ctx->stream2);
    if (ctx->seq_stream) (void)hipStreamSynchronize(ctx->seq_stream);
    ctx->cur = ctx->stream;
    (void)hipGetLastError();
    for (auto& r : ctx->prof_recs) prof_release(ctx, r);
    ctx->prof_recs.clear();
}

struct SlotLease {
    bbocr_ctx* root;
    bbocr_ctx* slot = nullptr;
    bool exclusive;
    SlotLease(bbocr_ctx* r, bool excl) : root(r), exclusive(excl) {
        std::unique_lock<std::mutex> lk(root->pool_mu);
        const int max_slots = root->cfg.call_slots == 1 ? 1 : kMaxSlots;
        if (exclusive) {
            root->pool_cv.wait(lk, [&] {
                if (root->slot_busy) return false;
                for (bbocr_ctx* s : root->slots) if (s->slot_busy) return false;
                return true;
            });
            root->slot_busy = true;
            for (bbocr_ctx* s : root->slots) s->slot_busy = true;
            slot = root;
            return;
        }
        for (;;) {
            if (!root->slot_busy) { slot = root; break; }
            for (bbocr_ctx* s : root->slots) if (!s->slot_busy) { slot = s; break; }
            if (slot) break;
            if ((int)root->slots.size() + 1 < max_slots) {
                slot = slot_create(root);
                root->slots.push_back(slot);
                break;
            }
            root->pool_cv.wait(lk);
        }
        slot->slot_busy = true;
        if (slot != root) {
            static_cast<WeightView&>(*slot) = static_cast<const WeightView&>(*root);
            slot->cfg = root->cfg;
            slot->cfg_beam_wide = root->cfg_beam_wide;
            slot->profiling = root->profiling;
        }
    }
    ~SlotLease() {
        {
            std::lock_guard<std::mutex> lk(root->pool_mu);
            if (exclusive) {
                root->slot_busy = false;
                for (bbocr_ctx* s : root->slots) s->slot_busy = false;
            } else if (slot) {
                slot->slot_busy = false;
            }
        }
        root->pool_cv.notify_all();
    }
};

inline void set_err(bbocr_ctx* root, const std::string& m) {
    std::lock_guard<std::mutex> lk(root->pool_mu);
    root->err = m;
}

template <typename F> inline int status_of(bbocr_ctx* root, F&& f) {
    if (!root) return BBOCR_ERR_ARG;
    try {
        f();
        return BBOCR_OK;
    } catch (const StatusError& se) {
        set_err(root, se.msg);
        return se.code;
    } catch (const std::exception& ex) {
        set_err(root, ex.what());
        return BBOCR_ERR_INTERNAL;
    } catch (...) {
        set_err(root, "unknown failure");
        return BBOCR_ERR_INTERNAL;
    }
}

template <typename F> inline int guarded(bbocr_ctx* root, F&& f, bool exclusive = false) {
    return status_of(root, [&] {
        HIPCHK(hipSetDevice(root->cfg.device));
        SlotLease lease(root, exclusive);
        bbocr_ctx* ctx = lease.slot;
        try {
            ctx->cur = ctx->stream;
            HIPCHK(hipStreamSynchronize(nullptr));
            f(ctx);
            publish_times(ctx);
        } catch (...) {
            guarded_drain(ctx);
            throw;
        }
    });
}

template <typename F> inline int lane_guarded(bbocr_ctx* root, SideLane bbocr_ctx::*which, bool wait_default, F&& f) {
    return status_of(root, [&] {
        HIPCHK(hipSetDevice(root->cfg.device));
        SideLane& lane = root->*which;
        std::lock_guard<std::mutex> lk(lane.mu);
        try {
            if (!lane.stream) HIPCHK(hipStreamCreateWithFlags(&lane.stream, hipStreamNonBlocking));
            if (wait_default) HIPCHK(hipStreamSynchronize(nullptr));
            f(lane.stream);
        } catch (...) {
            if (lane.stream) (void)hipStreamSynchronize(lane.stream);
            (void)hipGetLastError();
            throw;
        }
    });
}
```

### bb-ocr_amd/csrc/detector.cpp

```cpp
#include "ctx.h"

static hipEvent_t prof_event(bbocr_ctx* c) {
    hipEvent_t e;
    if (!c->prof_pool.empty()) { e = c->prof_pool.back(); c->prof_pool.pop_back(); }
    else HIPCHK(hipEventCreate(&e));
    return e;
}

template <typename F> static hipError_t profiled(bbocr_ctx* c, double flops, F&& launch) {
    if (c->profiling == 0 || (c->profiling == 1 && c->prof_group != 0)) return launch();
    bbocr_ctx::ProfRec r{prof_event(c), prof_event(c), flops, c->prof_group};
    HIPCHK(hipEventRecord(r.e0, c->cur));
    const hipError_t e = launch();
    HIPCHK(hipEventRecord(r.e1, c->cur));
    if (e == hipSuccess) c->prof_recs.push_back(r);
    else prof_release(c, r);
    return e;
}

hipError_t launch_conv_profiled(bbocr_ctx* c, const ConvPlan& p, ConvArgs a, bool may_decline) {
    a.zero = c->zero_page;
    const int OH = a.H + 2 * p.pad_h - (p.KH - 1) * p.dil, OW = a.W + 2 * p.pad_w - (p.KW - 1) * p.dil;
    double flops = 2.0 * a.N * OH * OW * (double)p.Cout * (p.split ? p.Cin / 3 : p.Cin) * p.KH * p.KW;
    if (a.c11_w) flops += 2.0 * a.N * a.H * a.W * 64.0 * 27.0;
    if (a.tail) flops += 2.0 * a.N * OH * OW * (16.0 * 16.0 + 16.0 * 2.0);
    if (a.post_w) flops += 2.0 * a.N * OH * OW * 64.0 * 64.0;
    const hipError_t e = profiled(c, flops, [&] { return launch_conv(p, a, c->cur); });
    if (may_decline && e == hipErrorNotSupported) return e;
    HIPCHK(e);
    return hipSuccess;
}

hipError_t launch_seq_proj_profiled(bbocr_ctx* c, const ConvPlan& p, const uint16_t* x, size_t rows_pad, uint16_t* out) {
    const double flops = 2.0 * (double)rows_pad * (double)p.Cout * p.Cin;
    const hipError_t e = profiled(c, flops, [&] { return launch_seq_proj(p, x, rows_pad, out, c->cur); });
    if (e != hipErrorNotSupported) HIPCHK(e);
    return e;
}

ConvArgs conv_args(const ConvPlan& p, const Act& a0, const Act* a1, const Act* addup) {
    ConvArgs a{};
    a.in0 = a0.p; a.C0 = a0.C; a.in0_cs = a0.C;
    a.N = a0.N; a.H = a0.H; a.W = a0.W;
    if (p.split) {
        if (a1 || (a0.C & 63)) fail(BBOCR_ERR_INTERNAL, "split-fp16 conv: one pair tensor with a multiple of 32 logical channels expected");
        a.in1 = a0.p; a.C1 = a0.C / 2; a.in1_cs = a0.C;
    } else if (a1) {
        a.in1 = a1->p; a.C1 = a1->C; a.in1_cs = a1->C;
    }
    if (addup) { a.addup = addup->p; a.up_H = a0.H; a.up_W = a0.W; a.up_cs = addup->C; }
    return a;
}

void run_conv(bbocr_ctx* c, const ConvPlan& p, const Act& a0, bool relu0, const Act* a1, bool relu1, bool relu_out, void* out,
                     int out_cs, int cout_store, bool out_f32, const Act* addup) {
    if (c->arena.dry) return;
    ConvArgs a = conv_args(p, a0, a1, addup);
    a.relu_in0 = relu0; a.relu_in1 = p.split ? relu0 : relu1; a.relu_out = relu_out; a.out_f32 = out_f32;
    a.out = out; a.out_cs = out_cs; a.cout_store = cout_store;
    if (p.split && !out_f32) a.split_off = cout_store;
    (void)launch_conv_profiled(c, p, a);
}

void prof_collect(bbocr_ctx* c) {
    bbocr_ctx* root = c->root;
    std::lock_guard<std::mutex> lk(root->pool_mu);
    for (auto& r : c->prof_recs) {
        float ms = 0.f;
        if (hipEventElapsedTime(&ms, r.e0, r.e1) == hipSuccess) {
            root->prof_ms[r.group] += ms;
            root->prof_flops[r.group] += r.flops;
            root->prof_launches[r.group] += 1;
        }
        prof_release(c, r);
    }
    c->prof_recs.clear();
}

static Act arena_act(bbocr_ctx* c, int N, int H, int W, int C) { return Act{c->arena.alloc<uint16_t>((size_t)N * H * W * C), N, H, W, C}; }

Act conv_act(bbocr_ctx* c, const ConvPlan& p, const Act& a0, bool relu0, const Act* a1, bool relu1, bool relu_out, int store) {
    const int OH = a0.H + 2 * p.pad_h - (p.KH - 1) * p.dil, OW = a0.W + 2 * p.pad_w - (p.KW - 1) * p.dil;
    const int cs = p.split ? 2 * store : store;
    Act o = arena_act(c, a0.N, OH, OW, cs);
    run_conv(c, p, a0, relu0, a1, relu1, relu_out, o.p, cs, store, false);
    return o;
}

Act conv_pool_act(bbocr_ctx* c, const ConvPlan& p, const Act& a0, bool relu0, bool relu_out, int store, int mode, bool pool_relu,
                         Act* full, const RgbSource* rgb) {
    const int OH = a0.H + 2 * p.pad_h - (p.KH - 1) * p.dil, OW = a0.W + 2 * p.pad_w - (p.KW - 1) * p.dil;
    const int PH = OH / 2, PW = mode == 1 ? OW / 2 : OW;
    const int cs = p.split ? 2 * store : store;
    if (full) *full = arena_act(c, a0.N, OH, OW, cs);
    Act o = arena_act(c, a0.N, PH, PW, cs);
    if (c->arena.dry) return o;
    ConvArgs a = conv_args(p, a0);
    a.relu_in0 = relu0; a.relu_in1 = relu0; a.relu_out = relu_out; a.out_f32 = 0;
    a.out = full ? (void*)full->p : nullptr; a.out_cs = cs; a.cout_store = store;
    if (p.split) a.split_off = store;
    a.pool_mode = mode; a.pool_relu = pool_relu; a.store_full = full != nullptr; a.pool_cs = cs; a.pool_out = o.p;
    if (rgb) { a.in0 = (const uint16_t*)rgb->rgb; a.c11_w = c->c11_wf; a.c11_b = c->c11_b; a.rgb_H = rgb->Himg; a.rgb_W = rgb->Wimg; }
    (void)launch_conv_profiled(c, p, a);
    return o;
}

Act pool_act(bbocr_ctx* c, const Act& a, int kh, int kw, int sh, int sw, int ph, int pw, bool relu_in) {
    const int OH = (a.H + 2 * ph - kh) / sh + 1, OW = (a.W + 2 * pw - kw) / sw + 1;
    Act o = arena_act(c, a.N, OH, OW, a.C);
    if (!c->arena.dry) HIPCHK(launch_maxpool(a.p, o.p, a.N, a.H, a.W, a.C, kh, kw, sh, sw, ph, pw, relu_in, c->cur));
    return o;
}


void craft_up_stage(bbocr_ctx* c, const ConvPlan& py, const ConvPlan& ps, const Act& y, const Act& skip, uint16_t* z, uint16_t* out) {
    const int cout = ps.Cout;
    const Act zz{z, y.N, y.H, y.W, cout};
    run_conv(c, py, y, false, nullptr, false, false, z, cout, cout, false);
    run_conv(c, ps, skip, false, nullptr, false, true, out, cout, cout, false, &zz);
}

bool craft_up3b_post(bbocr_ctx* c, const Act& u3a, uint16_t* u3b, uint16_t* z) {
    if (c->arena.dry) return false;
    if (c->up4y_post && !c->up3b.split) {
        ConvArgs a = conv_args(c->up3b, u3a);
        a.relu_out = 1; a.out = z; a.out_cs = 64; a.cout_store = 64; a.post_w = c->up4y_post;
        if (launch_conv_profiled(c, c->up3b, a, true) == hipSuccess) return true;
    }
    const Act b{u3b, u3a.N, u3a.H, u3a.W, 64};
    run_conv(c, c->up3b, u3a, false, nullptr, false, true, u3b, 64, 64, false);
    run_conv(c, c->up4y, b, false, nullptr, false, false, z, 64, 64, false);
    return false;
}

bool craft_up4(bbocr_ctx* c, const Act& s1, const uint16_t* z, uint16_t* u4b) {
    const Act zz{(uint16_t*)z, s1.N, s1.H / 2, s1.W / 2, 64};
    if (!c->arena.dry) {
        ConvArgs a = conv_args(c->up4s, s1, nullptr, &zz);
        a.relu_out = 1; a.out = u4b; a.out_cs = 32; a.cout_store = 32;
        a.zero = c->zero_page;
        const hipError_t e = profiled(c, 2.0 * a.N * a.H * a.W * (128.0 * 64.0 + 64.0 * 32.0 * 9.0), [&] { return launch_up4_fused(c->up4s, c->up4b, a, c->cur); });
        if (e == hipSuccess) return true;
        if (e != hipErrorNotSupported) HIPCHK(e);
    }
    Act u4a = arena_act(c, s1.N, s1.H, s1.W, 64);
    run_conv(c, c->up4s, s1, false, nullptr, false, true, u4a.p, 64, 64, false, &zz);
    run_conv(c, c->up4b, u4a, false, nullptr, false, true, u4b, 32, 32, false);
    return false;
}

void craft_cls_tail(bbocr_ctx* c, const Act& c2, float* heat) {
    if (c->arena.dry) return;
    ConvArgs a = conv_args(c->cls4, c2);
    a.relu_out = 1; a.out = heat; a.out_cs = 16; a.cout_store = 16; a.tail = c->cls_tail; a.tail_frag = c->cls_tail_frag;
    (void)launch_conv_profiled(c, c->cls4, a);
}

static void craft_forward(bbocr_ctx* c, const uint8_t* rgb, int nb, int Himg, int Wimg, int H32, int W32, float* heat) {
    c->prof_group = 0;
    const Act canvas{nullptr, nb, H32, W32, 64};
    const RgbSource src{rgb, Himg, Wimg};
    Act p1 = conv_pool_act(c, c->conv1_2, canvas, false, true, 64, 1, false, nullptr, &src);
    Act a3 = conv_act(c, c->conv2_1, p1, false, nullptr, false, true, 128);
    Act s1;
    Act p2 = conv_pool_act(c, c->conv2_2, a3, false, false, 128, 1, true, &s1);
    Act a5 = conv_act(c, c->conv3_1, p2, false, nullptr, false, true, 256);
    Act s2 = conv_act(c, c->conv3_2, a5, false, nullptr, false, false, 256);
    Act p3 = conv_pool_act(c, c->conv3_3, s2, true, true, 256, 1, false, nullptr);
    Act a8 = conv_act(c, c->conv4_1, p3, false, nullptr, false, true, 512);
    Act s3 = conv_act(c, c->conv4_2, a8, false, nullptr, false, false, 512);
    Act p4 = conv_pool_act(c, c->conv4_3, s3, true, true, 512, 1, false, nullptr);
    Act a11 = conv_act(c, c->conv5_1, p4, false, nullptr, false, true, 512);
    Act s4 = conv_act(c, c->conv5_2, a11, false, nullptr, false, false, 512);
    Act p5 = pool_act(c, s4, 3, 3, 1, 1, 1, 1, false);
    Act f6 = conv_act(c, c->fc6, p5, false, nullptr, false, false, 1024);
    Act f7 = conv_act(c, c->fc7, f6, false, nullptr, false, false, 1024);
    Act u1a = conv_act(c, c->up1a, f7, false, &s4, false, true, 512);
    Act u1b = conv_act(c, c->up1b, u1a, false, nullptr, false, true, 256);
    Act z2 = arena_act(c, u1b.N, u1b.H, u1b.W, 256), u2a = arena_act(c, s3.N, s3.H, s3.W, 256);
    craft_up_stage(c, c->up2y, c->up2s, u1b, s3, z2.p, u2a.p);
    Act u2b = conv_act(c, c->up2b, u2a, false, nullptr, false, true, 128);
    Act z3 = arena_act(c, u2b.N, u2b.H, u2b.W, 128), u3a = arena_act(c, s2.N, s2.H, s2.W, 128);
    craft_up_stage(c, c->up3y, c->up3s, u2b, s2, z3.p, u3a.p);
    Act u3b = arena_act(c, u3a.N, u3a.H, u3a.W, 64), z4 = arena_act(c, u3a.N, u3a.H, u3a.W, 64);
    (void)craft_up3b_post(c, u3a, u3b.p, z4.p);
    Act u4b = arena_act(c, s1.N, s1.H, s1.W, 32);
    (void)craft_up4(c, s1, z4.p, u4b.p);
    Act c1 = conv_act(c, c->cls0, u4b, false, nullptr, false, true, 32);
    Act c2 = conv_act(c, c->cls2, c1, false, nullptr, false, true, 32);
    craft_cls_tail(c, c2, heat);
}

static Act pair_act(bbocr_ctx* c, int N, int H, int W, int C) { return arena_act(c, N, H, W, 2 * C); }

static const ExactConvRow kExactConvs[] = {
    {"conv1_2", &bbocr_ctx::conv1_2, true, 64, 1, false, false},
    {"conv2_1", &bbocr_ctx::conv2_1, true, 128, 0, false, false},
    {"conv2_2", &bbocr_ctx::conv2_2, false, 128, 1, true, true},
    {"conv3_1", &bbocr_ctx::conv3_1, true, 256, 0, false, false},
    {"conv3_2", &bbocr_ctx::conv3_2, false, 256, 0, false, false},
    {"conv3_3", &bbocr_ctx::conv3_3, true, 256, 1, false, false},
    {"conv4_1", &bbocr_ctx::conv4_1, true, 512, 0, false, false},
    {"conv4_2", &bbocr_ctx::conv4_2, false, 512, 0, false, false},
    {"conv4_3", &bbocr_ctx::conv4_3, true, 512, 1, false, false},
    {"conv5_1", &bbocr_ctx::conv5_1, true, 512, 0, false, false},
    {"conv5_2", &bbocr_ctx::conv5_2, false, 512, 0, false, false},
    {"fc6", &bbocr_ctx::fc6, false, 1024, 0, false, false},
    {"fc7", &bbocr_ctx::fc7, false, 1024, 0, false, false},
    {"up1a", &bbocr_ctx::up1a, true, 512, 0, false, false},
    {"up1b", &bbocr_ctx::up1b, true, 256, 0, false, false},
    {"up2a", &bbocr_ctx::up2s, true, 256, 0, false, false},
    {"up2b", &bbocr_ctx::up2b, true, 128, 0, false, false},
    {"up3a", &bbocr_ctx::up3s, true, 128, 0, false, false},
    {"up3b", &bbocr_ctx::up3b, true, 64, 0, false, false},
    {"up4a", &bbocr_ctx::up4s, true, 64, 0, false, false},
    {"up4b", &bbocr_ctx::up4b, true, 32, 0, false, false},
    {"cls0", &bbocr_ctx::cls0, true, 32, 0, false, false},
    {"cls2", &bbocr_ctx::cls2, true, 32, 0, false, false},
    {"cls4", &bbocr_ctx::cls4, true, 16, 0, false, false},
};
int craft_exact_rows() { return (int)(sizeof(kExactConvs) / sizeof(kExactConvs[0])); }
const ExactConvRow& craft_exact_row(int row) {
    if (row < 0 || row >= craft_exact_rows()) fail(BBOCR_ERR_INTERNAL, "exact detector: no such conv row");
    return kExactConvs[row];
}

Act craft_exact_conv(bbocr_ctx* c, int row, const Act& in, Act* full) {
    const ExactConvRow& r = craft_exact_row(row);
    const ConvPlan& p = c->*(r.plan);
    if (r.keep_full != (full != nullptr)) fail(BBOCR_ERR_INTERNAL, "exact detector: a row keeps its full tensor exactly when the caller takes it");
    if (!r.pool_mode) return conv_act(c, p, in, false, nullptr, false, r.relu_out, r.store);
    return conv_pool_act(c, p, in, false, r.relu_out, r.store, r.pool_mode, r.pool_relu, full, nullptr);
}

Act craft_exact_conv1_1(bbocr_ctx* c, const uint8_t* rgb, int nb, int Himg, int Wimg, int H32, int W32) {
    Act o = pair_act(c, nb, H32, W32, 64);
    if (!c->arena.dry) HIPCHK(launch_pair_conv1_1(rgb, nb, Himg, Wimg, H32, W32, c->c11_w32, c->c11_b, o.p, c->cur));
    return o;
}
Act craft_exact_relu(bbocr_ctx* c, const Act& a) {
    Act o = pair_act(c, a.N, a.H, a.W, a.C / 2);
    if (!c->arena.dry) HIPCHK(launch_pair_relu(a.p, o.p, (size_t)a.N * a.H * a.W, a.C / 2, c->cur));
    return o;
}
Act craft_exact_upcat(bbocr_ctx* c, const Act& y, const Act& skip) {
    Act o = pair_act(c, skip.N, skip.H, skip.W, y.C / 2 + skip.C / 2);
    if (!c->arena.dry) HIPCHK(launch_pair_upcat(y.p, y.H, y.W, y.C / 2, skip.p, skip.C / 2, o.p, skip.N, skip.H, skip.W, c->cur));
    return o;
}
Act craft_exact_pool5(bbocr_ctx* c, const Act& s4) {
    Act o = pair_act(c, s4.N, s4.H, s4.W, s4.C / 2);
    if (!c->arena.dry) HIPCHK(launch_pair_maxpool3x3s1(s4.p, o.p, s4.N, s4.H, s4.W, s4.C / 2, c->cur));
    return o;
}
void craft_exact_cls_tail(bbocr_ctx* c, const Act& c3, float* heat) {
    if (c3.C != 32) fail(BBOCR_ERR_INTERNAL, "exact detector: the classifier tail reads a 16-channel pair");
    if (!c->arena.dry) HIPCHK(launch_pair_cls_tail(c3.p, c->cls6_w32, c->cls_tail, heat, (size_t)c3.N * c3.H * c3.W, c->cur));
}

static void craft_forward_exact(bbocr_ctx* c, const uint8_t* rgb, int nb, int Himg, int Wimg, int H32, int W32, float* heat) {
    c->prof_group = 0;
    int row = 0;
    auto conv = [&](const Act& a, Act* full = nullptr) { return craft_exact_conv(c, row++, a, full); };
    Act x0 = craft_exact_conv1_1(c, rgb, nb, Himg, Wimg, H32, W32);
    Act p1 = conv(x0);
    Act a3 = conv(p1);
    Act s1;
    Act p2 = conv(a3, &s1);
    Act a5 = conv(p2);
    Act s2 = conv(a5);
    Act p3 = conv(craft_exact_relu(c, s2));
    Act a8 = conv(p3);
    Act s3 = conv(a8);
    Act p4 = conv(craft_exact_relu(c, s3));
    Act a11 = conv(p4);
    Act s4 = conv(a11);
    Act f6 = conv(craft_exact_pool5(c, s4));
    Act f7 = conv(f6);
    Act u1a = conv(craft_exact_upcat(c, f7, s4));
    Act u1b = conv(u1a);
    Act u2a = conv(craft_exact_upcat(c, u1b, s3));
    Act u2b = conv(u2a);
    Act u3a = conv(craft_exact_upcat(c, u2b, s2));
    Act u3b = conv(u3a);
    Act u4a = conv(craft_exact_upcat(c, u3b, s1));
    Act u4b = conv(u4a);
    Act c3 = conv(conv(conv(u4b)));
    if (row != craft_exact_rows()) fail(BBOCR_ERR_INTERNAL, "exact detector: the pass and its conv table disagree");
    craft_exact_cls_tail(c, c3, heat);
}

static void craft_forward_any(bbocr_ctx* c, const uint8_t* rgb, int nb, int Himg, int Wimg, int H32, int W32, float* heat) {
    if (det_split(c)) craft_forward_exact(c, rgb, nb, Himg, Wimg, H32, W32, heat);
    else craft_forward(c, rgb, nb, Himg, Wimg, H32, W32, heat);
}

DetDims det_dims(int H, int W, int canvas, double mag) {
    DetDims d;
    double target = mag * (double)std::max(H, W);
    if (target > canvas) target = canvas;
    d.ratio = target / (double)std::max(H, W);
    d.th = (int)(H * d.ratio);
    d.tw = (int)(W * d.ratio);
    d.H32 = d.th % 32 ? d.th + (32 - d.th % 32) : d.th;
    d.W32 = d.tw % 32 ? d.tw + (32 - d.tw % 32) : d.tw;
    d.h = d.H32 / 2;
    d.w = d.W32 / 2;
    return d;
}

DetPlan det_plan(bbocr_ctx* c, int B, int H, int W, const bbocr_params& p, bool overlapped) {
    if (!c->craft_loaded) fail(BBOCR_ERR_STATE, "detector weights not loaded");
    if (B <= 0 || H <= 0 || W <= 0) fail(BBOCR_ERR_ARG, "bad page batch shape");
    DetPlan s;
    s.H = H; s.W = W;
    const DetDims d = s.d = det_dims(H, W, p.canvas_size, p.mag_ratio);
    if (d.th <= 0 || d.tw <= 0) fail(BBOCR_ERR_ARG, "page collapses to zero size");
    std::vector<int>& passes = s.passes;
    int sb_other = 0;
    if (c->cfg.det_sub_batch > 0) {
        for (int b0 = 0; b0 < B; b0 += c->cfg.det_sub_batch) passes.push_back(std::min(c->cfg.det_sub_batch, B - b0));
    } else {
        c->arena.begin(true);
        craft_forward_any(c, nullptr, 1, d.th, d.tw, d.H32, d.W32, nullptr);
        const size_t per_page = std::max<size_t>(c->arena.off, 1);
        const int cap = (int)std::max<size_t>(1, std::min<size_t>(64, ((size_t)96 << 30) / per_page));
        constexpr int kTailEquiv = 8;
        const double equiv = std::max(1.0, (double)d.th * d.tw / (960.0 * 1280.0));
        const int tail_pages = std::max(1, (int)std::lround(kTailEquiv / equiv));
        const bool alone = !other_call_in_flight(c);
        const int tail = (alone && overlapped && B * equiv >= 24.0 && cap > tail_pages && B > tail_pages) ? tail_pages : 0;
        const int body = B - tail, nbig = cdiv(body, cap);
        for (int i = 0; i < nbig; ++i) passes.push_back(body / nbig + (i < body % nbig ? 1 : 0));
        if (tail) passes.push_back(tail);
        sb_other = cdiv(B, cdiv(B, cap));
    }
    const int sb = std::max(sb_other, *std::max_element(passes.begin(), passes.end()));
    s.resized_bytes = (d.th != H || d.tw != W) ? (size_t)sb * d.th * d.tw * 3 : 0;
    c->arena.begin(true);
    craft_forward_any(c, nullptr, sb, d.th, d.tw, d.H32, d.W32, nullptr);
    s.arena_bytes = c->arena.off;
    return s;
}

void det_size(bbocr_ctx* c, size_t arena_bytes, size_t resized_bytes) {
    if (resized_bytes) c->resized.ensure(resized_bytes);
    c->arena.buf.ensure(arena_bytes);
}

void det_run(bbocr_ctx* c, const DetPlan& s, const uint8_t* rgb, float* heat, const std::function<void(int, int)>& after_sub) {
    const DetDims& d = s.d;
    int b0 = 0;
    for (const int nb : s.passes) {
        EnqLock enq(c);
        const uint8_t* src = rgb + (size_t)b0 * s.H * s.W * 3;
        if (s.resized_bytes) {
            HIPCHK(launch_resize_u8(src, nb, s.H, s.W, 3, (uint8_t*)c->resized.p, d.th, d.tw, c->stream));
            src = (const uint8_t*)c->resized.p;
        }
        c->arena.begin(false);
        craft_forward_any(c, src, nb, d.th, d.tw, d.H32, d.W32, heat + (size_t)b0 * d.h * d.w * 2);
        if (after_sub) after_sub(b0, nb);
        b0 += nb;
    }
}

void detect_impl(bbocr_ctx* c, const uint8_t* rgb, int B, int H, int W, const bbocr_params& p, float* heat,
                        const std::function<void(int, int)>& after_sub) {
    const DetPlan s = det_plan(c, B, H, W, p, after_sub != nullptr);
    det_size(c, s.arena_bytes, s.resized_bytes);
    det_run(c, s, rgb, heat, after_sub);
}


int ccl_cap_comps(int B, int h, int w) { return (int)std::min<size_t>(0x3fffffff, (size_t)B * ((size_t)h * w / 10 + 1)); }
void ccl_size(bbocr_ctx* c, size_t npx, int cap_comps) {
    c->ccl_label.ensure(npx * 4);
    c->ccl_stat.ensure(npx * 24);
    c->ccl_slot.ensure(npx * 4);
    c->ccl_comps.ensure((size_t)cap_comps * sizeof(CclOut));
    c->ccl_rowext.ensure(std::min<size_t>(0x3fffffff, npx) * 8);
    c->ccl_counters.ensure(16);
}

void boxes_impl(bbocr_ctx* c, const float* heat, int B, int h, int w, double ratio, const bbocr_params& p, HostBoxes& hb,
                       hipStream_t st) {
    if (B <= 0 || h <= 0 || w <= 0 || !(ratio > 0)) fail(BBOCR_ERR_ARG, "bad heat-map shape");
    const size_t npx = (size_t)B * h * w;
    const int cap_comps = ccl_cap_comps(B, h, w);
    const int cap_rows = (int)std::min<size_t>(0x3fffffff, npx);
    ccl_size(c, npx, cap_comps);
    if (!c->ccl_t0) { HIPCHK(hipEventCreate(&c->ccl_t0)); HIPCHK(hipEventCreate(&c->ccl_t1)); }
    HIPCHK(hipEventRecord(c->ccl_t0, st));
    HIPCHK(launch_ccl(heat, B, h, w, (float)p.low_text, (float)p.link_threshold, (double)p.text_threshold, (int*)c->ccl_label.p,
                      (int*)c->ccl_stat.p, (int*)c->ccl_slot.p, (CclOut*)c->ccl_comps.p, (int*)c->ccl_rowext.p, (int*)c->ccl_counters.p,
                      cap_comps, cap_rows, st));
    HIPCHK(hipEventRecord(c->ccl_t1, st));
    int counters[4] = {0, 0, 0, 0};
    HIPCHK(hipMemcpyAsync(counters, c->ccl_counters.p, sizeof(counters), hipMemcpyDeviceToHost, st));
    slot_sync(c, st);
    if (counters[2]) fail(BBOCR_ERR_OVERFLOW, "component buffers too small for this batch");
    std::vector<CclOut> all_comps(counters[0]);
    std::vector<int> all_rows((size_t)counters[1] * 2);
    if (counters[0]) HIPCHK(hipMemcpyAsync(all_comps.data(), c->ccl_comps.p, all_comps.size() * sizeof(CclOut), hipMemcpyDeviceToHost, st));
    if (counters[1]) HIPCHK(hipMemcpyAsync(all_rows.data(), c->ccl_rowext.p, all_rows.size() * 4, hipMemcpyDeviceToHost, st));
    slot_sync(c, st);
    std::vector<std::vector<CclOut>> comps(B);
    for (const CclOut& co : all_comps)
        if (co.img >= 0 && co.img < B) comps[co.img].push_back(co);
    float ccl_ms = 0.f;
    HIPCHK(hipEventElapsedTime(&ccl_ms, c->ccl_t0, c->ccl_t1));
    c->times[1] += ccl_ms;
    auto t0 = clk::now();
    const double ratio_w = 1.0 / ratio, ratio_h = 1.0 / ratio;
    bbocr::GroupParams gp{p.slope_ths, p.ycenter_ths, p.height_ths, p.width_ths, p.add_margin, p.min_size};
    hb.polys.assign(B, {});
    hb.hori.assign(B, {});
    hb.freeb.assign(B, {});
    auto do_page = [&](int b) {
        std::sort(comps[b].begin(), comps[b].end(), [](const CclOut& x, const CclOut& y) { return x.root < y.root; });
        for (const CclOut& co : comps[b]) {
            bbocr::Component cc{co.root, co.left, co.top, co.right, co.bottom, co.area, co.row_off};
            float box[4][2];
            bbocr::component_box(cc, all_rows.data() + (size_t)co.row_off * 2, w, h, box);
            std::array<int, 8> poly;
            bbocr::box_to_poly(box, ratio_w, ratio_h, poly.data());
            hb.polys[b].push_back(poly);
        }
        bbocr::group_text_box(hb.polys[b], gp, hb.hori[b], hb.freeb[b]);
    };
    host_pool(c).parallel_for(B, do_page);
    c->times[2] += (float)ms_since(t0);
}

bbocr_boxlist* export_boxes(const HostBoxes& hb) {
    const int B = (int)hb.polys.size();
    bbocr_boxlist* o = (bbocr_boxlist*)calloc(1, sizeof(bbocr_boxlist));
    o->n_images = B;
    o->poly_off = (int*)calloc(B + 1, sizeof(int));
    o->hori_off = (int*)calloc(B + 1, sizeof(int));
    o->free_off = (int*)calloc(B + 1, sizeof(int));
    for (int b = 0; b < B; ++b) {
        o->poly_off[b + 1] = o->poly_off[b] + (int)hb.polys[b].size();
        o->hori_off[b + 1] = o->hori_off[b] + (int)hb.hori[b].size();
        o->free_off[b + 1] = o->free_off[b] + (int)hb.freeb[b].size();
    }
    o->polys = (int*)calloc((size_t)std::max(1, o->poly_off[B]) * 8, sizeof(int));
    o->hori = (int*)calloc((size_t)std::max(1, o->hori_off[B]) * 4, sizeof(int));
    o->free_q = (double*)calloc((size_t)std::max(1, o->free_off[B]) * 8, sizeof(double));
    for (int b = 0; b < B; ++b) {
        for (size_t i = 0; i < hb.polys[b].size(); ++i) memcpy(o->polys + ((size_t)o->poly_off[b] + i) * 8, hb.polys[b][i].data(), 32);
        for (size_t i = 0; i < hb.hori[b].size(); ++i) memcpy(o->hori + ((size_t)o->hori_off[b] + i) * 4, hb.hori[b][i].data(), 16);
        for (size_t i = 0; i < hb.freeb[b].size(); ++i) memcpy(o->free_q + ((size_t)o->free_off[b] + i) * 8, hb.freeb[b][i].data(), 64);
    }
    return o;
}

void import_boxes(const bbocr_boxlist* bl, HostBoxes& hb) {
    const int B = bl->n_images;
    hb.polys.assign(B, {});
    hb.hori.assign(B, {});
    hb.freeb.assign(B, {});
    for (int b = 0; b < B; ++b) {
        for (int i = bl->hori_off[b]; i < bl->hori_off[b + 1]; ++i) {
            std::array<int, 4> a;
            memcpy(a.data(), bl->hori + (size_t)i * 4, 16);
            hb.hori[b].push_back(a);
        }
        for (int i = bl->free_off[b]; i < bl->free_off[b + 1]; ++i) {
            std::array<double, 8> a;
            memcpy(a.data(), bl->free_q + (size_t)i * 8, 64);
            hb.freeb[b].push_back(a);
        }
    }
}
```

### bb-ocr_amd/csrc/kernels.h

```cpp
#pragma once
#include <hip/hip_runtime.h>
#include <stdint.h>
#include <vector>

struct ConvArgs {
    const uint16_t* in0;
    const uint16_t* in1;
    const uint16_t* wpk;
    const float* bias;
    void* out;
    int C0, C1;
    int in0_cs, in1_cs;
    int N, H, W, OH, OW;
    int KH, KW, pad_h, pad_w, dil;
    int TH, TW, tiles_x, tiles_y, ntiles_n;
    int PH, PW, NP;
    int relu_in0, relu_in1, relu_out, out_f32;
    int out_cs, cout_store;
    int nchunks, ntaps;
    int pool_mode, pool_relu, store_full, pool_cs;
    void* pool_out;
    const uint16_t* aux_w;
    const float* tail;
    const uint16_t* tail_frag;
    const uint16_t* post_w;
    int sub;
    int stack;
    const void* zero;
    const uint16_t* addup;
    int up_H, up_W, up_cs;
    const uint16_t* c11_w;
    const float* c11_b;
    int rgb_H, rgb_W;
    const float* aux_b;
    float acc_scale;
    int lean;
    int split_off;
};

struct ConvPlan {
    int Cin = 0, Cout = 0;
    int Cin_pad = 0, Cout_pad = 0;
    int KH = 1, KW = 1, pad_h = 0, pad_w = 0, dil = 1;
    int BN = 64;
    int el = 0;
    float acc_scale = 1.f;
    int split = 0;
    uint16_t* d_w = nullptr;
    float* d_b = nullptr;
};

enum ConvRouteId : int {
    CONV_ROUTE_NONE = 0,
    CONV_ROUTE_GEN64_P4, CONV_ROUTE_GEN64_P8, CONV_ROUTE_GEN64_P16, CONV_ROUTE_GEN128_P4, CONV_ROUTE_GEN128_P8, CONV_ROUTE_GEN128_P16,
    CONV_ROUTE_DMA64_FUSE1, CONV_ROUTE_DMA64_POSTW,
    CONV_ROUTE_RESW_POOL64, CONV_ROUTE_RESW_1CH, CONV_ROUTE_RESW_2CH,
    CONV_ROUTE_DMA64_324_NF2, CONV_ROUTE_DMA64_324, CONV_ROUTE_DMA64_384, CONV_ROUTE_DMA64_448,
    CONV_ROUTE_DMA128_384, CONV_ROUTE_DMA128_448,
    CONV_ROUTE_DMA2X2_64, CONV_ROUTE_DMA2X2_128,
    CONV_ROUTE_DMA1X1_64, CONV_ROUTE_DMA1X1_128, CONV_ROUTE_DMA1X1_256, CONV_ROUTE_DMA1X1_ADDUP,
    CONV_ROUTE_COUNT
};
struct ConvRoute {
    int id;
    int status;
    int el, wm, wn, mf;
    int piter;
    int npb, ring, nps, fuse1, nf, epi, ks;
    int addup;
    int resw;
    int OH, OW, TH, TW, PH, PW, NP, sub, stack, tiles_x, tiles_y, ntiles_n, nchunks, ntaps, lean;
    int grid, threads;
    int persistent;
    int lds_bytes;
    int tail, split_off;
};

int conv_plan_bn(int Cout);
size_t conv_packed_elems(const ConvPlan& p);
void pack_conv_weights(const ConvPlan& p, const float* w, uint16_t* out);
hipError_t launch_conv(const ConvPlan& p, ConvArgs a, hipStream_t s, ConvRoute* route = nullptr, bool dry = false);
hipError_t launch_up4_fused(const ConvPlan& p1, const ConvPlan& p3, ConvArgs a, hipStream_t s);

void pack_post1x1_weights(const float* w , uint16_t* out , int el);
void pack_conv1_1_weights_fused(const float* w , uint16_t* out , int el);
hipError_t launch_maxpool(const uint16_t* in, uint16_t* out, int N, int H, int W, int C, int kh, int kw, int sh, int sw, int ph, int pw,
                          int relu_in, hipStream_t s);
hipError_t launch_gray(const uint8_t* rgb, uint8_t* gray, size_t npix, hipStream_t s);
__device__ __forceinline__ uint8_t bgr2gray_px(int c0, int c1, int c2) { return (uint8_t)((c2 * 9798 + c1 * 19235 + c0 * 3735 + (1 << 14)) >> 15); }
hipError_t launch_ycc_to_rgb_gray(const uint8_t* ycc, int stride, uint8_t* rgb, uint8_t* gray, size_t npix, hipStream_t s);
__device__ __forceinline__ void jpeg_ycc_to_rgb(int y, int cb, int cr, uint8_t* rgb) {
    cb -= 128;
    cr -= 128;
    int r = y + ((91881 * cr + 32768) >> 16);
    int g = y + ((-22554 * cb + 32768 - 46802 * cr) >> 16);
    int b = y + ((116130 * cb + 32768) >> 16);
    rgb[0] = (uint8_t)(r < 0 ? 0 : (r > 255 ? 255 : r));
    rgb[1] = (uint8_t)(g < 0 ? 0 : (g > 255 ? 255 : g));
    rgb[2] = (uint8_t)(b < 0 ? 0 : (b > 255 ? 255 : b));
}
hipError_t launch_resize_u8(const uint8_t* src, int N, int sh, int sw, int C, uint8_t* dst, int dh, int dw, hipStream_t s);

hipError_t launch_pair_conv1_1(const uint8_t* rgb, int N, int Hi, int Wi, int H, int W, const float* w , const float* b, uint16_t* out,
                               hipStream_t s);
hipError_t launch_pair_relu(const uint16_t* in, uint16_t* out, size_t npix, int C, hipStream_t s);
hipError_t launch_pair_maxpool3x3s1(const uint16_t* in, uint16_t* out, int N, int H, int W, int C, hipStream_t s);
hipError_t launch_pair_upcat(const uint16_t* y, int yh, int yw, int Cy, const uint16_t* skip, int Cs, uint16_t* out, int N, int H, int W, hipStream_t s);
hipError_t launch_pair_cls_tail(const uint16_t* in , const float* w1 , const float* tail , float* heat,
                                size_t npix, hipStream_t s);

struct CclOut {
    int root, left, top, right, bottom, area, row_off, img;
};
hipError_t launch_ccl(const float* heat, int N, int h, int w, float low_text, float link_thr, double text_thr, int* label, int* stat,
                      int* slot, CclOut* comps, int* rowext, int* counters, int cap_comps, int cap_rows, hipStream_t s);

struct CropDesc {
    int img;
    int sx0, sy0, sw, sh;
    int rw, rh;
    int fw;
    int imgW;
    int slot;
    int warp;
    int warp_off;
    int a_off;
    int lut_off;
    int pad_;
    int rot;
    double Minv[9];
};
struct CropPage {
    long long off;
    long long pitch;
    int H, W;
};
hipError_t launch_crops(const uint8_t* gray, int H, int W, const CropDesc* descs_dev, int first, int count, int imgW, int any_warp,
                        int any_tall, uint8_t* wscratch, uint8_t* scratch, uint8_t* hscratch, const uint8_t* luts, uint16_t* out_bucket,
                        int stage_mask, hipStream_t s, int wide_row_stride = 0, int gap = 0, int mode = 0,
                        const CropPage* pages = nullptr);
enum { REC_BF16 = 0, REC_F16 = 1, REC_SPLIT = 2 };
constexpr float SPLIT_LO_SCALE = 2048.f;
hipError_t launch_crop_hist(const uint8_t* scratch, const CropDesc* descs_dev, int first, int count, unsigned int* hist, hipStream_t s);
hipError_t launch_crnn_conv0(const uint16_t* in, const float* w , const float* b, uint16_t* out, int n, int W, int mode, hipStream_t s,
                             const uint16_t* afrag = nullptr );
void pack_crnn_conv0_mfma(const float* w_tap_major , uint16_t* out , int el);
hipError_t launch_crnn_zero_gaps(uint16_t* t, const CropDesc* descs_dev, int first, int count, int H, int Wl, int C, int shift, hipStream_t s);
hipError_t launch_rowmean3_gather(const uint16_t* in, int Wc, int C, const CropDesc* descs_dev, int first, int count, uint16_t* out, int mode,
                                  hipStream_t s);
hipError_t launch_lstm(const void* xproj, const uint16_t* whh_pk, uint16_t* out, const int* tiles_dev, int ntiles, int mode, float acc_scale,
                       hipStream_t s);
int lstm_tile_seqs(int mode);
size_t lstm_whh_packed_elems();
void pack_lstm_whh8(const float* whh_fwd, const float* whh_bwd, uint16_t* out, int el);
size_t lstm_whh_split_packed_elems();
float pack_lstm_whh_split(const float* whh_fwd, const float* whh_bwd, uint16_t* out);
int lstm8_xproj_channel(int dir, int gate, int unit);
struct SeqProjPlan { int grid, chunks, ring; long long nslots, chunk_slots; };
SeqProjPlan seq_proj_plan(size_t rows_pad, int ncu);
hipError_t launch_seq_proj(const ConvPlan& p, const uint16_t* x, size_t rows_pad, uint16_t* out, hipStream_t s);
size_t q8_packed_bytes(int N, int K);
void pack_q8_weights(const int8_t* q , int N, int K, int8_t* out);
void pack_q8_whh(const int8_t* q_fwd, const int8_t* q_bwd , int8_t* out );
hipError_t launch_q8_quantize(const void* x, int src_pair, int K, size_t rows, size_t rows_pad, const int* seqs_dev, int nseq, float* rowp, int8_t* a8,
                              uint8_t* codes, float* segp, hipStream_t s);
hipError_t launch_q8_gemm(const int8_t* a8, size_t rows_pad, int K, const int8_t* wpk, int N, const float* rowp, const float* wscale, const float* bias,
                          float* out, int ldo, hipStream_t s);
constexpr int LSTM_Q8_SEQS = 16;
hipError_t launch_lstm_q8(const float* G, const int8_t* whh_pk, const float* whh_scale, const float* bhh, float* out, const int* seqs_dev,
                          const int* tiles_dev, int ntiles, float* c_out, uint8_t* hcodes, float* hparams, hipStream_t s);
struct CtcOut { int len; int cnt; float prod; int pad; };
hipError_t launch_ctc(const float* logits, size_t rows, int C, int cs, const int* seqs_dev, int nseq, int* idx_tmp, float* pmax_tmp,
                      int* out_idx, CtcOut* out, hipStream_t s, const unsigned int* ignore = nullptr, float* probs_out = nullptr);
hipError_t launch_ctc_wide(const float* logits, size_t rows, int C, int cs, const int* seqs_dev, int nseq, int* idx_tmp, float* pmax_tmp,
                           int* out_idx, CtcOut* out, hipStream_t s, const unsigned int* mask_dev = nullptr, float* probs_out = nullptr);
hipError_t launch_ctc_collapse(const int* idx, const float* pmax, const int* seqs_dev, int nseq, int* out_idx, CtcOut* out, hipStream_t s);
constexpr int kPredCtcRows = 64;
size_t pred_ctc_packed_elems(int C);
size_t pred_ctc_bias_elems(int C);
void pack_pred_ctc_weights(int el, const float* w , const float* b , int C, uint16_t* wpk, float* bias);
hipError_t launch_pred_ctc(int el, const uint16_t* x, size_t rows, const uint16_t* wpk, const float* bias, int C, const unsigned int* mask_dev,
                           int* idx, float* pmax, hipStream_t s);
void ctc_beam_search_host(const float* mat, int T, int C, int cs, int beam_width, std::vector<int>& text);
class HostPool;
void ctc_beam_search_batch(const float* probs, const int* seqs, int nseq, int C, int cs, int beam_width, std::vector<std::vector<int>>& texts,
                           HostPool* pool = nullptr);
constexpr size_t kCtcBeamLdsLimit = 65536;
size_t ctc_beam_lds_bytes(int beam_width, int C, int max_T);
bool ctc_beam_on_device(int beam_width, int C, int max_T);
hipError_t launch_ctc_beam(const float* probs, size_t rows, int C, int cs, const int* seqs_dev, int nseq, int max_T, int beam_width, int* out_text,
                           int* out_len, hipStream_t s);
constexpr int kBeamWideCand = 128;
size_t ctc_beam_wide_lds_bytes(int beam_width, int max_T);
bool ctc_beam_wide_on_device(int beam_width, int C, int max_T);
hipError_t launch_ctc_beam_wide(const float* probs, size_t rows, int C, int cs, const int* seqs_dev, int nseq, int max_T, int beam_width, int* cand_n,
                                int* cand, int* out_text, int* out_len, hipStream_t s);

int pp_resize_tile_rows(int H, int W, int dh, int dw);
hipError_t launch_pp_resize_cubic(const uint8_t* src, int H, int W, uint8_t* dst, int dh, int dw, const int* x0, const double* wx, const long long* nx,
                                  const int* y0, const double* wy, const long long* ny, unsigned long long KX, unsigned long long KY, hipStream_t s, int src_bgr = 0);
hipError_t launch_pp_gauss3(const uint8_t* src, int H, int W, uint8_t* dst, int k0, int k1, int k2, unsigned long long* sum, hipStream_t s);
hipError_t launch_pp_clahe_hist(const uint8_t* src, int H, int W, const uint8_t* lut, int tw, int th, int tx, int ty, unsigned int* hist,
                                hipStream_t s);
hipError_t launch_pp_clahe_apply(const uint8_t* src, int H, int W, const uint8_t* lut, const uint8_t* tile_luts, int tw, int th, int tx, int ty,
                                 uint8_t* dst, hipStream_t s);
hipError_t launch_pp_box_pass(const uint8_t* src, uint8_t* dst, int H, int W, int vertical, int r, unsigned int ww, unsigned int fw, hipStream_t s);
hipError_t launch_pp_fold_lut(const unsigned long long* sum, unsigned long long n, float contrast, float brightness, uint8_t* lut, hipStream_t s);
hipError_t launch_pp_clahe_luts(const unsigned int* hist, int tiles, int clip, float lut_scale, uint8_t* tile_luts, hipStream_t s);
hipError_t launch_pp_lut(const uint8_t* src, uint8_t* dst, const uint8_t* lut, size_t total, hipStream_t s);
bool pp_unsharp_fused_ok(int H, int W, int r, const uint8_t* a, const uint8_t* b, const uint8_t* c);
hipError_t launch_pp_unsharp_fused(const uint8_t* in, uint8_t* tmp, uint8_t* dst, int H, int W, unsigned int ww, unsigned int fw, int percent,
                                   int threshold, hipStream_t s);
hipError_t launch_pp_unsharp(const uint8_t* in, const uint8_t* blur, uint8_t* dst, size_t total, int percent, int threshold, hipStream_t s);

constexpr int AC_BOX = 35, AC_BOX_R = 17, AC_MEAN_C = 10;
constexpr int AC_GAU = 31, AC_GAU_R = 15, AC_GAU_C = 5;
struct AcTaps { int k[AC_GAU]; };
hipError_t launch_ac_gray_blur(const uint8_t* src, int H, int W, size_t pitch, int channels, uint8_t* dst, hipStream_t s);
hipError_t launch_ac_cues(const uint8_t* e, int H, int W, const AcTaps& taps, uint16_t* rbox, uint16_t* rgau, uint8_t* part, uint8_t* grad,
                          unsigned int* hist, int* thr, hipStream_t s);
hipError_t launch_ac_pack(const uint8_t* e, const uint8_t* part, const uint8_t* grad, const int* thr, int H, int W, int WW, uint32_t* bits, hipStream_t s);
hipError_t launch_ac_pack_mask(const uint8_t* src, size_t pitch, int H, int W, int WW, uint32_t* bits, hipStream_t s);
hipError_t launch_ac_rect(const uint32_t* src, uint32_t* tmp, uint32_t* dst, int H, int W, int WW, int rx, int ry, int erode, const uint32_t* or_with,
                          hipStream_t s);
hipError_t launch_ac_components(const uint32_t* bits, int H, int W, int WW, int* label, uint8_t* flag, int* count, int cap, int* boxes, hipStream_t s);
hipError_t launch_ac_unpack(const uint32_t* bits, const int* label, int H, int W, int WW, uint8_t* dst, hipStream_t s);

enum : int { PAGE_GRAY = 0, PAGE_BGR = 1, PAGE_RGB = 2, PAGE_YCC4 = 3, PAGE_YCC3 = 4 };
__host__ __device__ constexpr int page_px_bytes(int layout) { return layout == PAGE_GRAY ? 1 : (layout == PAGE_YCC4 ? 4 : 3); }

constexpr int PK_TILE_PX = 4096;
constexpr int PK_MAX_TILES = (1 << 24) - 1;
struct PackPage {
    const uint8_t* rgb;
    const uint8_t* gray;
    long long rgb_pitch, gray_pitch;
    long long rgb_off, gray_off;
    int H, W;
    int tile0;
    int vec;
};
int pack_page_vec(const PackPage& g, const uint8_t* rgb_staging, const uint8_t* gray_staging);
hipError_t launch_pack_pages(const PackPage* pages_dev, int n, int ntiles, uint8_t* rgb_staging, uint8_t* gray_staging, hipStream_t s);

constexpr int TH_PRECISION_BITS = 22;
struct ThQuant { unsigned short q[2][64]; };
hipError_t launch_th_reduce(const uint8_t* src, size_t pitch, int layout, int H, int W, int fx, int fy, uint8_t* dst, int rh, int rw, int C,
                            hipStream_t s);
hipError_t launch_th_resample_h(const uint8_t* src, size_t pitch, int layout, int y0, int rows, int ow, int C, const int* bounds, const int* kk,
                                int ksize, uint8_t* dst, hipStream_t s);
hipError_t launch_th_resample_v(const uint8_t* src, size_t spitch, int y0, int width, int oh, const int* bounds, const int* kk, int ksize,
                                uint8_t* dst, size_t dpitch, hipStream_t s);
hipError_t launch_th_jpeg(const uint8_t* src, size_t pitch, int C, int H, int W, const ThQuant& q, uint8_t* yp, int wp, uint8_t* cbp, uint8_t* crp,
                          hipStream_t s);
hipError_t launch_th_upsample(const uint8_t* yp, int wp, const uint8_t* cbp, const uint8_t* crp, int H, int W, int gray_only, uint8_t* rgb,
                              uint8_t* gray, uint8_t* ycc, hipStream_t s);
hipError_t launch_th_direct(const uint8_t* src, size_t pitch, int layout, int H, int W, uint8_t* rgb, uint8_t* gray, hipStream_t s);

constexpr int JE_TILE = 256;
constexpr int JE_STUFF_TILE = 2048;
constexpr int JE_BLOCK_MAX_BITS = 22 + 63 * 26;
struct JeHuff { uint32_t dc[2][16], ac[2][256]; };
struct JeStdTable { unsigned char bits[16], vals[162]; int n; };
constexpr JeStdTable JE_STD[4] = {
    {{0, 1, 5, 1, 1, 1, 1, 1, 1, 0, 0, 0, 0, 0, 0, 0}, {0, 1, 2, 3, 4, 5, 6, 7, 8, 9, 10, 11}, 12},
    {{0, 2, 1, 3, 3, 2, 4, 3, 5, 5, 4, 4, 0, 0, 1, 0x7D},
     {0x01, 0x02, 0x03, 0x00, 0x04, 0x11, 0x05, 0x12, 0x21, 0x31, 0x41, 0x06, 0x13, 0x51, 0x61, 0x07, 0x22, 0x71, 0x14, 0x32, 0x81, 0x91, 0xA1,
      0x08, 0x23, 0x42, 0xB1, 0xC1, 0x15, 0x52, 0xD1, 0xF0, 0x24, 0x33, 0x62, 0x72, 0x82, 0x09, 0x0A, 0x16, 0x17, 0x18, 0x19, 0x1A, 0x25, 0x26,
      0x27, 0x28, 0x29, 0x2A, 0x34, 0x35, 0x36, 0x37, 0x38, 0x39, 0x3A, 0x43, 0x44, 0x45, 0x46, 0x47, 0x48, 0x49, 0x4A, 0x53, 0x54, 0x55, 0x56,
      0x57, 0x58, 0x59, 0x5A, 0x63, 0x64, 0x65, 0x66, 0x67, 0x68, 0x69, 0x6A, 0x73, 0x74, 0x75, 0x76, 0x77, 0x78, 0x79, 0x7A, 0x83, 0x84, 0x85,
      0x86, 0x87, 0x88, 0x89, 0x8A, 0x92, 0x93, 0x94, 0x95, 0x96, 0x97, 0x98, 0x99, 0x9A, 0xA2, 0xA3, 0xA4, 0xA5, 0xA6, 0xA7, 0xA8, 0xA9, 0xAA,
      0xB2, 0xB3, 0xB4, 0xB5, 0xB6, 0xB7, 0xB8, 0xB9, 0xBA, 0xC2, 0xC3, 0xC4, 0xC5, 0xC6, 0xC7, 0xC8, 0xC9, 0xCA, 0xD2, 0xD3, 0xD4, 0xD5, 0xD6,
      0xD7, 0xD8, 0xD9, 0xDA, 0xE1, 0xE2, 0xE3, 0xE4, 0xE5, 0xE6, 0xE7, 0xE8, 0xE9, 0xEA, 0xF1, 0xF2, 0xF3, 0xF4, 0xF5, 0xF6, 0xF7, 0xF8, 0xF9,
      0xFA}, 162},
    {{0, 3, 1, 1, 1, 1, 1, 1, 1, 1, 1, 0, 0, 0, 0, 0}, {0, 1, 2, 3, 4, 5, 6, 7, 8, 9, 10, 11}, 12},
    {{0, 2, 1, 2, 4, 4, 3, 4, 7, 5, 4, 4, 0, 1, 2, 0x77},
     {0x00, 0x01, 0x02, 0x03, 0x11, 0x04, 0x05, 0x21, 0x31, 0x06, 0x12, 0x41, 0x51, 0x07, 0x61, 0x71, 0x13, 0x22, 0x32, 0x81, 0x08, 0x14, 0x42,
      0x91, 0xA1, 0xB1, 0xC1, 0x09, 0x23, 0x33, 0x52, 0xF0, 0x15, 0x62, 0x72, 0xD1, 0x0A, 0x16, 0x24, 0x34, 0xE1, 0x25, 0xF1, 0x17, 0x18, 0x19,
      0x1A, 0x26, 0x27, 0x28, 0x29, 0x2A, 0x35, 0x36, 0x37, 0x38, 0x39, 0x3A, 0x43, 0x44, 0x45, 0x46, 0x47, 0x48, 0x49, 0x4A, 0x53, 0x54, 0x55,
      0x56, 0x57, 0x58, 0x59, 0x5A, 0x63, 0x64, 0x65, 0x66, 0x67, 0x68, 0x69, 0x6A, 0x73, 0x74, 0x75, 0x76, 0x77, 0x78, 0x79, 0x7A, 0x82, 0x83,
      0x84, 0x85, 0x86, 0x87, 0x88, 0x89, 0x8A, 0x92, 0x93, 0x94, 0x95, 0x96, 0x97, 0x98, 0x99, 0x9A, 0xA2, 0xA3, 0xA4, 0xA5, 0xA6, 0xA7, 0xA8,
      0xA9, 0xAA, 0xB2, 0xB3, 0xB4, 0xB5, 0xB6, 0xB7, 0xB8, 0xB9, 0xBA, 0xC2, 0xC3, 0xC4, 0xC5, 0xC6, 0xC7, 0xC8, 0xC9, 0xCA, 0xD2, 0xD3, 0xD4,
      0xD5, 0xD6, 0xD7, 0xD8, 0xD9, 0xDA, 0xE2, 0xE3, 0xE4, 0xE5, 0xE6, 0xE7, 0xE8, 0xE9, 0xEA, 0xF2, 0xF3, 0xF4, 0xF5, 0xF6, 0xF7, 0xF8, 0xF9,
      0xFA}, 162},
};
constexpr JeHuff je_std_huff() {
    JeHuff h{};
    for (int t = 0; t < 4; ++t) {
        uint32_t* out = (t & 1) ? h.ac[t >> 1] : h.dc[t >> 1];
        uint32_t code = 0;
        int k = 0;
        for (int len = 1; len <= 16; ++len) {
            for (int i = 0; i < JE_STD[t].bits[len - 1]; ++i) out[JE_STD[t].vals[k++]] = (code++ << 5) | (uint32_t)len;
            code <<= 1;
        }
    }
    return h;
}
inline int je_blocks(int H, int W, int components) {
    return components == 1 ? ((H + 7) / 8) * ((W + 7) / 8) : 6 * ((H + 15) / 16) * ((W + 15) / 16);
}
hipError_t launch_je_coef(const uint8_t* src, size_t pitch, int layout, int components, int H, int W, const ThQuant& q, short* coef, hipStream_t s);
hipError_t launch_je_sizes(const short* coef, int n, int components, unsigned int* local, unsigned long long* tile_bits, hipStream_t s);
hipError_t launch_je_scan(unsigned long long* v, int n, hipStream_t s);
hipError_t launch_je_offsets(const unsigned int* local, const unsigned long long* tile_off, int n, long long* out, hipStream_t s);
hipError_t launch_je_pack(const short* coef, int n, int components, const unsigned int* local, const unsigned long long* tile_off, uint32_t* words,
                          hipStream_t s);
hipError_t launch_je_ff_count(const uint8_t* scan, long long bytes, unsigned long long* tile_ff, hipStream_t s);
hipError_t launch_je_stuff(const uint8_t* scan, long long bytes, const unsigned long long* tile_off, uint8_t* out, hipStream_t s);

constexpr int PNG_CHUNK = 16384;
constexpr int PNG_LITLEN = 286, PNG_CL = 19;
constexpr int PNG_HIST_ROW = 288;
constexpr int PNG_REC = 320;
constexpr int PNG_STORED = 0, PNG_DYNAMIC = 1;
constexpr int PNG_LIMIT15 = 1, PNG_LIMIT7 = 2;
struct PngRec {
    uint8_t kind, flags;
    uint8_t litlen[PNG_LITLEN];
    uint8_t dist;
    uint8_t cl[PNG_CL];
    uint8_t pad[PNG_REC - 2 - PNG_LITLEN - 1 - PNG_CL];
};
static_assert(sizeof(PngRec) == PNG_REC, "PngRec layout");
hipError_t launch_png_filter(const uint8_t* src, size_t pitch, int layout, int H, int W, uint8_t* stream, hipStream_t s);
hipError_t launch_png_codes(const uint8_t* stream, size_t n, int chunks, uint32_t* hist, PngRec* rec, unsigned long long* size, uint32_t* adler,
                            hipStream_t s);
hipError_t launch_png_pack(const uint8_t* stream, size_t n, int chunks, const PngRec* rec, const unsigned long long* off, uint8_t* out, hipStream_t s);

constexpr int ORIENT_TILE = 64;
bool page_orient_pair_ok(int layout, int dst_layout);
hipError_t launch_page_orient(const uint8_t* src, int H, int W, size_t pitch, int layout, int orientation, int dst_layout, uint8_t* dst,
                              size_t dst_pitch, hipStream_t s);

constexpr int JD_LANES = 64;
constexpr int JD_SUBSEQ_BITS = 1024;
struct JpegHuff {
    unsigned short look[512];
    int maxcode[18];
    int valoff[18];
    unsigned char val[256];
};
enum : int { JD_UP_NONE = 0, JD_UP_H2V1_FANCY = 1, JD_UP_H1V2_FANCY = 2, JD_UP_H2V2_NOT_NEEDED = 3, JD_UP_REPLICATE = 4, JD_UP_H2V2_FANCY = 5 };
struct JpegComp {
    int n;
    int bw, bh;
    int plane_rows, pitch;
    int valid_rows, valid_cols;
    int up;
};
struct JpegSubs {
    const uint8_t* data;
    const int* seg_byte;
    const int* seg_sub;
    const int* sub_seg;
    unsigned long long* entry;
    unsigned long long* exits;
    int* count;
    int* scan;
    int* flags;
    int nseg, nsub, S, passes;
};
struct JpegDesc : JpegSubs {
    int* first;
    int* status;
    short* coef;
    uint8_t* plane[3];
    uint8_t* out;
    long long pitch;
    JpegComp comp[3];
    int OW, OH;
    const JpegHuff* huff;
    const unsigned short* quant;
    int W, H, ncomp, bpm, mcux, mcuy, nmcu, ri, nblocks, px;
    int hs, vs;
    int tab_dc[3], tab_ac[3];
};
enum : int { JD_ERR_SYNC = 1, JD_ERR_CODE = 2, JD_ERR_COUNT = 4 };
hipError_t launch_jd_sync(const JpegDesc* descs, int n, int max_groups, int pass, hipStream_t s);
hipError_t launch_jd_scan(const JpegDesc* descs, int n, hipStream_t s);
hipError_t launch_jd_write(const JpegDesc* descs, int n, int max_groups, hipStream_t s);
hipError_t launch_jd_dc(const JpegDesc* descs, int n, int max_seg, hipStream_t s);
hipError_t launch_jd_idct(const JpegDesc* descs, int n, int max_blocks, hipStream_t s);
hipError_t launch_jd_output(const JpegDesc* descs, int n, int max_h, int max_w, hipStream_t s);
```

Baseline: 961.8.

## Restructure CCL into compact root list with wave-aggregated accept and vectorised crop writes

Rewrites the connected-component labelling pipeline. Each thread now handles four pixels, and the divisions become magic-number divmods. Stats are initialised only at run starts, and the roots are compacted into a list so the accept kernel scans only roots instead of every pixel. The accept kernel batches its atomics per wavefront, and slot/comps lookups in rowext are replaced by storing the component index and row offset inside stat. The crop final kernel also gets a normalisation LUT in shared memory, 4-wide vector stores, and a configurable block count. This adds complexity and new invariants: stat entries must only be read at roots, and lane-0 boundary handling in merge changes.

```diff
diff --git a/bb-ocr_amd/csrc/abi.cpp b/bb-ocr_amd/csrc/abi.cpp
--- a/bb-ocr_amd/csrc/abi.cpp
+++ b/bb-ocr_amd/csrc/abi.cpp
@@ -87,7 +87,7 @@
     if (c->seq_t1) { (void)hipEventDestroy(c->seq_t1); (void)hipEventDestroy(c->seq_t2); }
     for (auto& r : c->prof_recs) { (void)hipEventDestroy(r.e0); (void)hipEventDestroy(r.e1); }
     for (hipEvent_t e : c->prof_pool) (void)hipEventDestroy(e);
-    DevBuf* bufs[] = {&c->arena.buf, &c->heat, &c->gray, &c->resized, &c->ccl_label, &c->ccl_stat, &c->ccl_slot, &c->ccl_comps, &c->ccl_rowext,
+    DevBuf* bufs[] = {&c->arena.buf, &c->heat, &c->gray, &c->resized, &c->ccl_label, &c->ccl_stat, &c->ccl_roots, &c->ccl_comps, &c->ccl_rowext,
                       &c->ccl_counters, &c->crop_desc, &c->crop_desc2, &c->crop_scratch, &c->crop_hscratch, &c->crop_wscratch, &c->crop_luts, &c->crop_hist,
                       &c->ctc_idx, &c->ctc_pmax, &c->ctc_out_idx, &c->ctc_out, &c->seq_v, &c->seq_xp, &c->seq_h, &c->seq_lin, &c->seq_logits,
                       &c->seq_tables, &c->pp_gray, &c->pp_a, &c->pp_b, &c->pp_c, &c->pp_tab, &c->ctc_probs, &c->ctc_beam_idx, &c->ctc_beam_len, &c->ctc_cand, &c->ctc_cand_n, &c->ac_work, &c->th_coef, &c->je_scan, &c->je_out, &c->pe_out,
diff --git a/bb-ocr_amd/csrc/ccl.hip b/bb-ocr_amd/csrc/ccl.hip
--- a/bb-ocr_amd/csrc/ccl.hip
+++ b/bb-ocr_amd/csrc/ccl.hip
@@ -1,5 +1,15 @@
 #include "common.h"
 #include "kernels.h"
+
+constexpr int CCL_STAT = 6;
+constexpr int CCL_ACCEPT_BLOCKS = 256;
+
+__device__ __forceinline__ void ccl_divmod(unsigned i, unsigned d, unsigned m, unsigned& q, unsigned& r) {
+    q = __umulhi(i, m);
+    r = i - q * d;
+    if (r >= d) { r -= d; ++q; }
+}
+static unsigned ccl_magic(unsigned d) { return d <= 1 ? 0xffffffffu : (unsigned)(0x100000000ULL / d); }
 
 __device__ __forceinline__ int ccl_find(const int* __restrict__ label, int x) {
     int p = __hip_atomic_load(label + x, __ATOMIC_RELAXED, __HIP_MEMORY_SCOPE_AGENT);
@@ -22,19 +32,25 @@
     }
 }
 
-__global__ void __launch_bounds__(256) ccl_init_kernel(const float* __restrict__ heat, size_t total, int w, float low_text, float link_thr,
-                                                       int* __restrict__ label, int* __restrict__ stat, int* __restrict__ slot) {
-    const int lane = threadIdx.x & 63;
-    const size_t nround = (total + (size_t)gridDim.x * 256 - 1) / ((size_t)gridDim.x * 256);
-    for (size_t it = 0; it < nround; ++it) {
-        const size_t i = (it * gridDim.x + blockIdx.x) * 256 + threadIdx.x;
-        bool fg = false;
-        int x = 0;
-        if (i < total) {
-            const float2 v = *(const float2*)(heat + i * 2);
-            fg = (v.x > low_text) || (v.y > link_thr);
-            x = (int)(i % w);
-        }
+constexpr int CCL_K = 4;
+
+__global__ void __launch_bounds__(256) ccl_init_kernel(const float* __restrict__ heat, unsigned total, unsigned w, unsigned mw, float low_text,
+                                                       float link_thr, int* __restrict__ label, int* __restrict__ stat) {
+    const int lane = threadIdx.x & 63;
+    const unsigned i0 = blockIdx.x * (256u * CCL_K) + threadIdx.x;
+    float2 v[CCL_K];
+#pragma unroll
+    for (int k = 0; k < CCL_K; ++k) {
+        const unsigned i = i0 + k * 256u;
+        v[k] = make_float2(0.f, 0.f);
+        if (i < total) v[k] = *(const float2*)(heat + (size_t)i * 2);
+    }
+#pragma unroll
+    for (int k = 0; k < CCL_K; ++k) {
+        const unsigned i = i0 + k * 256u;
+        const bool fg = i < total && ((v[k].x > low_text) || (v[k].y > link_thr));
+        unsigned q, x;
+        ccl_divmod(i, w, mw, q, x);
         const unsigned long long fgm = __ballot(fg);
         const bool start = fg && (lane == 0 || x == 0 || !((fgm >> (lane - 1)) & 1ULL));
         const unsigned long long sm = __ballot(start);
@@ -45,136 +61,222 @@
                 lab = (int)i - (lane - (63 - __clzll((long long)below)));
             }
             label[i] = lab;
-            slot[i] = -1;
-            int* st = stat + i * 6;
-            st[0] = 0x7fffffff; st[1] = -1; st[2] = 0x7fffffff; st[3] = -1; st[4] = 0; st[5] = 0;
-        }
-    }
-}
-
-__global__ void __launch_bounds__(256) ccl_merge_kernel(size_t total, int h, int w, int* label) {
-    for (size_t i = (size_t)blockIdx.x * 256 + threadIdx.x; i < total; i += (size_t)gridDim.x * 256) {
-        if (label[i] < 0) continue;
-        const int x = (int)(i % w);
-        const int y = (int)((i / w) % h);
-        const bool left = x > 0 && label[i - 1] >= 0;
-        if (left && (i & 63) == 0) ccl_union(label, (int)i, (int)i - 1);
-        if (y > 0 && label[i - w] >= 0 && !(left && label[i - w - 1] >= 0)) ccl_union(label, (int)i, (int)i - w);
-    }
-}
-
-__global__ void __launch_bounds__(256) ccl_stats_kernel(const float* __restrict__ heat, size_t total, int h, int w, int* label,
-                                                        int* __restrict__ stat) {
-    const int lane = threadIdx.x & 63;
-    const size_t nround = (total + (size_t)gridDim.x * 256 - 1) / ((size_t)gridDim.x * 256);
-    for (size_t it = 0; it < nround; ++it) {
-        const size_t i = (it * gridDim.x + blockIdx.x) * 256 + threadIdx.x;
-        int r = -1, x = 0, y = 0;
-        float t = 0.f;
-        if (i < total && label[i] >= 0) {
-            r = ccl_find(label, (int)i);
+            if (start) {
+                int2* st = (int2*)(stat + (size_t)i * CCL_STAT);
+                st[0] = make_int2(0x7fffffff, -1);
+                st[1] = make_int2(0x7fffffff, -1);
+                st[2] = make_int2(0, 0);
+            }
+        }
+    }
+}
+
+__global__ void __launch_bounds__(256) ccl_merge_kernel(unsigned total, unsigned h, unsigned w, unsigned mh, unsigned mw, int* label) {
+    const int lane = threadIdx.x & 63;
+    const unsigned i0 = blockIdx.x * (256u * CCL_K) + threadIdx.x;
+    int lab[CCL_K], up[CCL_K];
+    unsigned xs[CCL_K], ys[CCL_K];
+#pragma unroll
+    for (int k = 0; k < CCL_K; ++k) {
+        const unsigned i = i0 + k * 256u;
+        unsigned row, q;
+        ccl_divmod(i, w, mw, row, xs[k]);
+        ccl_divmod(row, h, mh, q, ys[k]);
+        lab[k] = -1; up[k] = -1;
+        if (i < total) {
+            lab[k] = label[i];
+            if (ys[k] > 0) up[k] = label[i - w];
+        }
+    }
+#pragma unroll
+    for (int k = 0; k < CCL_K; ++k) {
+        const unsigned i = i0 + k * 256u;
+        int lf = __shfl_up(lab[k], 1), ul = __shfl_up(up[k], 1);
+        if (lab[k] < 0) continue;
+        const unsigned x = xs[k], y = ys[k];
+        if (lane == 0 && x > 0) {
+            lf = label[i - 1];
+            ul = y > 0 ? label[i - w - 1] : -1;
+        }
+        const bool left = x > 0 && lf >= 0;
+        if (left && lane == 0) ccl_union(label, (int)i, (int)i - 1);
+        if (y > 0 && up[k] >= 0 && !(left && ul >= 0)) ccl_union(label, (int)i, (int)(i - w));
+    }
+}
+
+__global__ void __launch_bounds__(256) ccl_stats_kernel(const float* __restrict__ heat, unsigned total, unsigned h, unsigned w, unsigned mh,
+                                                        unsigned mw, int* label, int* __restrict__ stat, int* __restrict__ roots,
+                                                        int* counters) {
+    const int lane = threadIdx.x & 63;
+    const unsigned i0 = blockIdx.x * (256u * CCL_K) + threadIdx.x;
+    int lab[CCL_K];
+    float ts[CCL_K];
+#pragma unroll
+    for (int k = 0; k < CCL_K; ++k) {
+        const unsigned i = i0 + k * 256u;
+        lab[k] = i < total ? label[i] : -1;
+    }
+#pragma unroll
+    for (int k = 0; k < CCL_K; ++k) {
+        const unsigned i = i0 + k * 256u;
+        ts[k] = lab[k] >= 0 ? fmaxf(heat[(size_t)i * 2], 0.f) : 0.f;
+    }
+#pragma unroll
+    for (int k = 0; k < CCL_K; ++k) {
+        const unsigned i = i0 + k * 256u;
+        int r = -1;
+        unsigned x = 0, y = 0;
+        const float t = ts[k];
+        if (lab[k] >= 0) {
+            r = ccl_find(label, lab[k]);
             label[i] = r;
-            x = (int)(i % w);
-            y = (int)((i / w) % h);
-            t = fmaxf(heat[i * 2], 0.f);
+            unsigned row, q;
+            ccl_divmod(i, w, mw, row, x);
+            ccl_divmod(row, h, mh, q, y);
+        }
+        const unsigned long long rm = __ballot(r == (int)i);
+        if (rm) {
+            int base = 0;
+            if (lane == 0) base = atomicAdd(counters + 3, __popcll(rm));
+            base = __shfl(base, 0);
+            if (r == (int)i) roots[base + __popcll(rm & ((1ULL << lane) - 1ULL))] = r;
         }
         const int rp = __shfl_up(r, 1);
         const bool head = r >= 0 && (lane == 0 || rp != r || x == 0);
         const unsigned long long hm = __ballot(head || r < 0);
-        if (r >= 0) {
-            const unsigned long long below = hm & ((lane == 63) ? ~0ULL : ((1ULL << (lane + 1)) - 1ULL));
-            const int first = 63 - __clzll((long long)below);
-            const unsigned long long above = (lane == 63) ? 0ULL : (hm >> (lane + 1));
-            const int len_after = above ? (__ffsll((long long)above) - 1) : (63 - lane);
-            float m = t;
+        const unsigned long long above = (lane == 63) ? 0ULL : (hm >> (lane + 1));
+        const int len_after = above ? (__ffsll((long long)above) - 1) : (63 - lane);
+        float m = t;
+#pragma unroll
+        for (int o = 1; o < 64; o <<= 1) {
+            const float mo = __shfl_down(m, o);
+            if (o <= len_after) m = fmaxf(m, mo);
+        }
+        if (head) {
+            int* st = stat + (size_t)r * CCL_STAT;
+            atomicMin(st + 0, (int)x);
+            atomicMax(st + 1, (int)x + len_after);
+            atomicMin(st + 2, (int)y);
+            atomicMax(st + 3, (int)y);
+            atomicAdd(st + 4, len_after + 1);
+            if (m > 0.f) atomicMax(st + 5, __float_as_int(m));
+        }
+    }
+}
+
+__global__ void __launch_bounds__(256) ccl_accept_kernel(unsigned hw, unsigned mhw, double text_thr, const int* __restrict__ roots,
+                                                         int* __restrict__ stat, CclOut* comps, int* rowext, int* counters, int cap_comps,
+                                                         int cap_rows) {
+    const int lane = threadIdx.x & 63;
+    const int n = counters[3];
+    const int stride = gridDim.x * 256;
+    for (int k0 = blockIdx.x * 256 + (threadIdx.x & ~63); k0 < n; k0 += stride) {
+        const int k = k0 + lane;
+        bool ok = false;
+        int root = 0, hh = 0, area = 0;
+        int* st = nullptr;
+        if (k < n) {
+            root = roots[k];
+            st = stat + (size_t)root * CCL_STAT;
+            area = st[4];
+            ok = area >= 10 && !((double)__int_as_float(st[5]) < text_thr);
+            if (ok) hh = st[3] - st[2] + 1;
+        }
+        const unsigned long long am = __ballot(ok);
+        if (am) {
+            int incl = hh;
 #pragma unroll
             for (int o = 1; o < 64; o <<= 1) {
-                const float mo = __shfl_down(m, o);
-                if (o <= len_after) m = fmaxf(m, mo);
-            }
-            if (head) {
-                int* st = stat + (size_t)r * 6;
-                atomicMin(st + 0, x);
-                atomicMax(st + 1, x + len_after);
-                atomicMin(st + 2, y);
-                atomicMax(st + 3, y);
-                atomicAdd(st + 4, len_after + 1);
-                if (m > 0.f) atomicMax(st + 5, __float_as_int(m));
-            }
-            (void)first;
-        }
-    }
-}
-
-__global__ void __launch_bounds__(256) ccl_accept_kernel(size_t total, int hw, double text_thr, const int* __restrict__ label,
-                                                         const int* __restrict__ stat, int* __restrict__ slot, CclOut* comps,
-                                                         int* rowext, int* counters, int cap_comps, int cap_rows) {
-    for (size_t i = (size_t)blockIdx.x * 256 + threadIdx.x; i < total; i += (size_t)gridDim.x * 256) {
-        if (label[i] != (int)i) continue;
-        const int* st = stat + i * 6;
-        const int area = st[4];
-        if (area < 10) continue;
-        if ((double)__int_as_float(st[5]) < text_thr) continue;
-        const int img = (int)(i / hw);
-        const int hh = st[3] - st[2] + 1;
-        const int idx = atomicAdd(counters + 0, 1);
-        const int off = atomicAdd(counters + 1, hh);
-        if (idx >= cap_comps || off + hh > cap_rows) { atomicOr(counters + 2, 1); continue; }
-        CclOut c;
-        c.root = (int)(i - (size_t)img * hw);
-        c.left = st[0]; c.top = st[2]; c.right = st[1]; c.bottom = st[3]; c.area = area; c.row_off = off; c.img = img;
-        comps[idx] = c;
-        slot[i] = idx;
-        int* re = rowext + (size_t)off * 2;
-        for (int k = 0; k < hh; ++k) { re[2 * k] = 0x7fffffff; re[2 * k + 1] = -1; }
-    }
-}
-
-__global__ void __launch_bounds__(256) ccl_rowext_kernel(const float* __restrict__ heat, size_t total, int h, int w, float low_text,
-                                                         const int* __restrict__ label, const int* __restrict__ slot,
-                                                         const CclOut* __restrict__ comps, int* rowext, int cap_comps, int cap_rows) {
-    const int lane = threadIdx.x & 63;
-    const size_t nround = (total + (size_t)gridDim.x * 256 - 1) / ((size_t)gridDim.x * 256);
-    for (size_t it = 0; it < nround; ++it) {
-        const size_t i = (it * gridDim.x + blockIdx.x) * 256 + threadIdx.x;
-        int r = -1, x = 0;
-        if (i < total) {
-            r = label[i];
-            if (r >= 0 && !(heat[i * 2] > low_text)) r = -1;
-            x = (int)(i % w);
-        }
+                const int v = __shfl_up(incl, o);
+                if (lane >= o) incl += v;
+            }
+            const int rows = __shfl(incl, 63);
+            int idx0 = 0, off0 = 0;
+            if (lane == 0) {
+                idx0 = atomicAdd(counters + 0, __popcll(am));
+                off0 = atomicAdd(counters + 1, rows);
+            }
+            idx0 = __shfl(idx0, 0);
+            off0 = __shfl(off0, 0);
+            const int idx = idx0 + __popcll(am & ((1ULL << lane) - 1ULL));
+            const int off = off0 + incl - hh;
+            if (ok && (idx >= cap_comps || off + hh > cap_rows)) { atomicOr(counters + 2, 1); ok = false; }
+            if (ok) {
+                unsigned img, in_img;
+                ccl_divmod((unsigned)root, hw, mhw, img, in_img);
+                CclOut c;
+                c.root = (int)in_img;
+                c.left = st[0]; c.top = st[2]; c.right = st[1]; c.bottom = st[3]; c.area = area; c.row_off = off; c.img = (int)img;
+                comps[idx] = c;
+                st[4] = idx;
+                st[5] = off - c.top;
+            }
+            int2* re = (int2*)rowext;
+            for (int j = lane; j < rows && off0 + j < cap_rows; j += 64) re[(size_t)off0 + j] = make_int2(0x7fffffff, -1);
+        }
+        if (k < n && !ok) st[4] = -1;
+    }
+}
+
+__global__ void __launch_bounds__(256) ccl_rowext_kernel(const float* __restrict__ heat, unsigned total, unsigned h, unsigned w, unsigned mh,
+                                                         unsigned mw, float low_text, const int* __restrict__ label,
+                                                         const int* __restrict__ stat, int* rowext) {
+    const int lane = threadIdx.x & 63;
+    const unsigned i0 = blockIdx.x * (256u * CCL_K) + threadIdx.x;
+    int lab[CCL_K];
+    float ts[CCL_K];
+#pragma unroll
+    for (int k = 0; k < CCL_K; ++k) {
+        const unsigned i = i0 + k * 256u;
+        lab[k] = i < total ? label[i] : -1;
+    }
+#pragma unroll
+    for (int k = 0; k < CCL_K; ++k) {
+        const unsigned i = i0 + k * 256u;
+        ts[k] = lab[k] >= 0 ? heat[(size_t)i * 2] : 0.f;
+    }
+#pragma unroll
+    for (int k = 0; k < CCL_K; ++k) {
+        const unsigned i = i0 + k * 256u;
+        int r = lab[k];
+        if (r >= 0 && !(ts[k] > low_text)) r = -1;
+        if (!__ballot(r >= 0)) continue;
+        unsigned row, x;
+        ccl_divmod(i, w, mw, row, x);
         const int rp = __shfl_up(r, 1);
         const bool head = r >= 0 && (lane == 0 || rp != r || x == 0);
         const unsigned long long hm = __ballot(head || r < 0);
         if (head) {
-            const int s = slot[r];
-            if (s >= 0) {
+            const int2 sb = *(const int2*)(stat + (size_t)r * CCL_STAT + 4);
+            if (sb.x >= 0) {
                 const unsigned long long above = (lane == 63) ? 0ULL : (hm >> (lane + 1));
                 const int len_after = above ? (__ffsll((long long)above) - 1) : (63 - lane);
-                const CclOut c = comps[s];
-                const int y = (int)((i / w) % h);
-                int* re = rowext + ((size_t)c.row_off + (y - c.top)) * 2;
-                atomicMin(re, x);
-                atomicMax(re + 1, x + len_after);
+                unsigned q, y;
+                ccl_divmod(row, h, mh, q, y);
+                int* re = rowext + (size_t)(sb.y + (int)y) * 2;
+                atomicMin(re, (int)x);
+                atomicMax(re + 1, (int)x + len_after);
             }
         }
     }
 }
 
 hipError_t launch_ccl(const float* heat, int N, int h, int w, float low_text, float link_thr, double text_thr, int* label, int* stat,
-                      int* slot, CclOut* comps, int* rowext, int* counters, int cap_comps, int cap_rows, hipStream_t s) {
-    const size_t total = (size_t)N * h * w;
-    if (total == 0) return hipSuccess;
-    if (total > 0x7fffffffULL) return hipErrorInvalidValue;
-    const int grid = (int)((total + 255) / 256 < 16384 ? (total + 255) / 256 : 16384);
+                      int* roots, CclOut* comps, int* rowext, int* counters, int cap_comps, int cap_rows, hipStream_t s) {
+    const size_t total64 = (size_t)N * h * w;
+    if (total64 == 0) return hipSuccess;
+    if (total64 > 0x7fffffffULL) return hipErrorInvalidValue;
+    const unsigned total = (unsigned)total64, uh = (unsigned)h, uw = (unsigned)w, hw = uh * uw;
+    const unsigned mh = ccl_magic(uh), mw = ccl_magic(uw), mhw = ccl_magic(hw);
+    const int grid = (int)((total + 256u * CCL_K - 1u) / (256u * CCL_K));
+    const int agrid = grid < CCL_ACCEPT_BLOCKS ? grid : CCL_ACCEPT_BLOCKS;
     hipError_t e = hipMemsetAsync(counters, 0, sizeof(int) * 4, s);
     if (e != hipSuccess) return e;
-    hipLaunchKernelGGL(ccl_init_kernel, dim3(grid), dim3(256), 0, s, heat, total, w, low_text, link_thr, label, stat, slot);
-    hipLaunchKernelGGL(ccl_merge_kernel, dim3(grid), dim3(256), 0, s, total, h, w, label);
-    hipLaunchKernelGGL(ccl_stats_kernel, dim3(grid), dim3(256), 0, s, heat, total, h, w, label, stat);
-    hipLaunchKernelGGL(ccl_accept_kernel, dim3(grid), dim3(256), 0, s, total, h * w, text_thr, label, stat, slot, comps, rowext, counters,
-                       cap_comps, cap_rows);
-    hipLaunchKernelGGL(ccl_rowext_kernel, dim3(grid), dim3(256), 0, s, heat, total, h, w, low_text, label, slot, comps, rowext, cap_comps,
+    hipLaunchKernelGGL(ccl_init_kernel, dim3(grid), dim3(256), 0, s, heat, total, uw, mw, low_text, link_thr, label, stat);
+    hipLaunchKernelGGL(ccl_merge_kernel, dim3(grid), dim3(256), 0, s, total, uh, uw, mh, mw, label);
+    hipLaunchKernelGGL(ccl_stats_kernel, dim3(grid), dim3(256), 0, s, heat, total, uh, uw, mh, mw, label, stat, roots, counters);
+    hipLaunchKernelGGL(ccl_accept_kernel, dim3(agrid), dim3(256), 0, s, hw, mhw, text_thr, roots, stat, comps, rowext, counters, cap_comps,
                        cap_rows);
+    hipLaunchKernelGGL(ccl_rowext_kernel, dim3(grid), dim3(256), 0, s, heat, total, uh, uw, mh, mw, low_text, label, stat, rowext);
     return hipGetLastError();
 }
diff --git a/bb-ocr_amd/csrc/crnn_misc.hip b/bb-ocr_amd/csrc/crnn_misc.hip
--- a/bb-ocr_amd/csrc/crnn_misc.hip
+++ b/bb-ocr_amd/csrc/crnn_misc.hip
@@ -16,8 +16,10 @@
     }
     uint8_t* dst = wscratch + d.warp_off;
     const int total = d.sw * d.sh;
-    for (int i = blockIdx.x * 256 + threadIdx.x; i < total; i += gridDim.x * 256) {
-        const int x = i % d.sw, y = i / d.sw;
+    const int step = gridDim.x * 256, step_y = step / d.sw, step_x = step - step_y * d.sw;
+    int i = blockIdx.x * 256 + threadIdx.x, y = i / d.sw, x = i - y * d.sw;
+    for (; i < total; i += step, x += step_x, y += step_y) {
+        if (x >= d.sw) { x -= d.sw; ++y; }
         const double X0 = d.Minv[0] * (double)x + (d.Minv[1] * (double)y + d.Minv[2]);
         const double Y0 = d.Minv[3] * (double)x + (d.Minv[4] * (double)y + d.Minv[5]);
         const double W0 = d.Minv[6] * (double)x + (d.Minv[7] * (double)y + d.Minv[8]);
@@ -53,46 +55,73 @@
     s1 = sx + 1 < ssize ? sx + 1 : ssize - 1;
 }
 
+constexpr int CROP_BLOCKS = 16;
+constexpr int CROP_YTAB = 256;
+
 template <bool PAGES>
 __global__ void __launch_bounds__(256) crop_resize_kernel(const uint8_t* __restrict__ gray, int H, int W, const CropDesc* __restrict__ descs,
                                                           int first, const uint8_t* __restrict__ wscratch, uint8_t* __restrict__ scratch,
                                                           const CropPage* __restrict__ pages) {
-    const CropDesc d = descs[first + blockIdx.y];
+    __shared__ int4 ytab[CROP_YTAB];
+    const CropDesc& dd = descs[first + blockIdx.y];
+    const int rot = dd.rot, sw = dd.sw, sh = dd.sh, dw = (rot & 1) ? dd.rh : dd.rw, dh = (rot & 1) ? dd.rw : dd.rh;
+    const long long want = ((long long)dw * dh + 256 * 4 - 1) / (256 * 4);
+    const int nb = want < 1 ? 1 : (want > (long long)gridDim.x ? (int)gridDim.x : (int)want);
+    if ((int)blockIdx.x >= nb) return;
+    const bool same = (dw == sw && dh == sh), area2 = (sw == 2 * dw && sh == 2 * dh), lin = !same && !area2;
+    const double scale_x = 1.0 / ((double)dw / (double)sw), scale_y = 1.0 / ((double)dh / (double)sh);
+    const bool tab = lin && dh <= CROP_YTAB;
+    if (tab) {
+        if ((int)threadIdx.x < dh) {
+            int y0, y1, b0, b1;
+            cv_lin_coef_d((int)threadIdx.x, sh, scale_y, y0, y1, b0, b1);
+            ytab[threadIdx.x] = make_int4(y0, y1, b0, b1);
+        }
+        __syncthreads();
+    }
+    const int T = nb * 256, t = blockIdx.x * 256 + threadIdx.x;
+    int rstep = 1, rphase = 0, c0 = t, cstep = T;
+    if (T >= dw) {
+        rstep = T / dw; rphase = t / dw; c0 = t - rphase * dw; cstep = dw;
+        if (rphase >= rstep) return;
+    }
     const uint8_t* src;
     size_t stride;
-    if (d.warp) { src = wscratch + d.warp_off; stride = (size_t)d.sw; }
+    if (dd.warp) { src = wscratch + dd.warp_off; stride = (size_t)sw; }
     else if constexpr (PAGES) {
-        const CropPage pg = pages[d.img];
-        src = gray + pg.off + (size_t)d.sy0 * (size_t)pg.pitch + d.sx0; stride = (size_t)pg.pitch;
-    }
-    else { src = gray + (size_t)d.img * H * W + (size_t)d.sy0 * W + d.sx0; stride = (size_t)W; }
-    uint8_t* dst = scratch + d.a_off;
-    const int sw = d.sw, sh = d.sh, dw = (d.rot & 1) ? d.rh : d.rw, dh = (d.rot & 1) ? d.rw : d.rh;
-    const bool same = (dw == sw && dh == sh), area2 = (sw == 2 * dw && sh == 2 * dh);
-    const double scale_x = 1.0 / ((double)dw / (double)sw), scale_y = 1.0 / ((double)dh / (double)sh);
-    const int total = dw * dh;
-    for (int i = blockIdx.x * 256 + threadIdx.x; i < total; i += gridDim.x * 256) {
-        const int dx = i % dw, dy = i / dw;
-        int v;
-        if (same) {
-            v = src[(size_t)dy * stride + dx];
-        } else if (area2) {
-            v = (src[(size_t)(2 * dy) * stride + 2 * dx] + src[(size_t)(2 * dy) * stride + 2 * dx + 1] +
-                 src[(size_t)(2 * dy + 1) * stride + 2 * dx] + src[(size_t)(2 * dy + 1) * stride + 2 * dx + 1] + 2) >> 2;
-        } else {
-            int x0, x1, a0, a1, y0, y1, b0, b1;
-            cv_lin_coef_d(dx, sw, scale_x, x0, x1, a0, a1);
-            cv_lin_coef_d(dy, sh, scale_y, y0, y1, b0, b1);
-            const int r0 = src[(size_t)y0 * stride + x0] * a0 + src[(size_t)y0 * stride + x1] * a1;
-            const int r1 = src[(size_t)y1 * stride + x0] * a0 + src[(size_t)y1 * stride + x1] * a1;
-            v = (((b0 * (r0 >> 4)) >> 16) + ((b1 * (r1 >> 4)) >> 16) + 2) >> 2;
-            v = v < 0 ? 0 : (v > 255 ? 255 : v);
-        }
-        int o = i;
-        if (d.rot == 1) o = (dw - 1 - dx) * dh + dy;
-        else if (d.rot == 2) o = (dh - 1 - dy) * dw + (dw - 1 - dx);
-        else if (d.rot == 3) o = dx * dh + (dh - 1 - dy);
-        dst[o] = (uint8_t)v;
+        const CropPage pg = pages[dd.img];
+        src = gray + pg.off + (size_t)dd.sy0 * (size_t)pg.pitch + dd.sx0; stride = (size_t)pg.pitch;
+    }
+    else { src = gray + (size_t)dd.img * H * W + (size_t)dd.sy0 * W + dd.sx0; stride = (size_t)W; }
+    uint8_t* dst = scratch + dd.a_off;
+    for (int dx = c0; dx < dw; dx += cstep) {
+        int x0 = 0, x1 = 0, a0 = 0, a1 = 0;
+        if (lin) cv_lin_coef_d(dx, sw, scale_x, x0, x1, a0, a1);
+#pragma unroll 2
+        for (int dy = rphase; dy < dh; dy += rstep) {
+            int v;
+            if (same) {
+                v = src[(size_t)dy * stride + dx];
+            } else if (area2) {
+                v = (src[(size_t)(2 * dy) * stride + 2 * dx] + src[(size_t)(2 * dy) * stride + 2 * dx + 1] +
+                     src[(size_t)(2 * dy + 1) * stride + 2 * dx] + src[(size_t)(2 * dy + 1) * stride + 2 * dx + 1] + 2) >> 2;
+            } else {
+                int y0, y1, b0, b1;
+                if (tab) { const int4 c = ytab[dy]; y0 = c.x; y1 = c.y; b0 = c.z; b1 = c.w; }
+                else cv_lin_coef_d(dy, sh, scale_y, y0, y1, b0, b1);
+                const uint8_t* s0 = src + (size_t)y0 * stride;
+                const uint8_t* s1 = src + (size_t)y1 * stride;
+                const int r0 = s0[x0] * a0 + s0[x1] * a1;
+                const int r1 = s1[x0] * a0 + s1[x1] * a1;
+                v = (((b0 * (r0 >> 4)) >> 16) + ((b1 * (r1 >> 4)) >> 16) + 2) >> 2;
+                v = v < 0 ? 0 : (v > 255 ? 255 : v);
+            }
+            int o = dy * dw + dx;
+            if (rot == 1) o = (dw - 1 - dx) * dh + dy;
+            else if (rot == 2) o = (dh - 1 - dy) * dw + (dw - 1 - dx);
+            else if (rot == 3) o = dx * dh + (dh - 1 - dy);
+            dst[o] = (uint8_t)v;
+        }
     }
 }
 
@@ -177,40 +206,77 @@
 __global__ void __launch_bounds__(256) crop_final_kernel(const CropDesc* __restrict__ descs, int first, const uint8_t* __restrict__ scratch,
                                                          const uint8_t* __restrict__ hscratch, const uint8_t* __restrict__ luts,
                                                          uint16_t* __restrict__ out, int row_stride, long long slot_stride, int gap) {
-    const CropDesc d = descs[first + blockIdx.y];
-    const bool tall = !(d.fw == d.rw && d.rh == 64);
-    const uint8_t* src = (tall ? hscratch : scratch) + d.a_off;
-    const uint8_t* lut = (!tall && d.lut_off >= 0) ? luts + d.lut_off : nullptr;
-    uint16_t* dst = out + (size_t)d.slot * (size_t)slot_stride;
-    const int imgW = d.imgW;
+    const CropDesc& dd = descs[first + blockIdx.y];
+    const int imgW = dd.imgW, fw = dd.fw, rw = dd.rw, rh = dd.rh;
+    const int ng = (imgW + gap + 3) >> 2;
+    int lg = 2;
+    while (lg < 6 && (1 << lg) < ng) ++lg;
     const int t = blockIdx.x * 256 + threadIdx.x;
-    const int y = t >> 6, x0 = t & 63;
+    const int y = t >> lg, g0 = t & ((1 << lg) - 1);
     if (y >= 64) return;
-    const bool vert = tall && d.rh != 64;
+    __shared__ uint16_t norm[256];
+    if constexpr (MODE != REC_SPLIT) {
+        norm[threadIdx.x] = El<MODE == REC_F16 ? 1 : 0>::from_f32(((float)(int)threadIdx.x / 255.0f - 0.5f) / 0.5f);
+        __syncthreads();
+    }
+    const bool tall = !(fw == rw && rh == 64);
+    const uint8_t* src = (tall ? hscratch : scratch) + dd.a_off;
+    const uint8_t* lut = (!tall && dd.lut_off >= 0) ? luts + dd.lut_off : nullptr;
+    const size_t base = (size_t)dd.slot * (size_t)slot_stride;
+    uint16_t* drow = out + base + (size_t)y * row_stride;
+    const bool wide_ok = !(((base | (size_t)row_stride | (size_t)imgW | (size_t)gap) & 3) || ((uintptr_t)out & 7));
+    const bool vert = tall && rh != 64;
     PilWin win;
-    if (vert) win = pil_window(d.rh, 64, y);
-    auto sample = [&](int xs) {
+    if (vert) win = pil_window(rh, 64, y);
+    auto conv = [&](int v) -> uint16_t {
+        if constexpr (MODE == REC_SPLIT) return (unsigned short)(v + 1);
+        else return norm[v];
+    };
+    auto sample = [&](int xs) -> uint16_t {
         int v;
         if (!tall) {
-            v = src[(size_t)y * d.rw + xs];
+            v = src[(size_t)y * rw + xs];
             if (lut) v = lut[v];
         } else if (!vert) {
-            v = src[(size_t)y * d.fw + xs];
+            v = src[(size_t)y * fw + xs];
         } else {
             long long acc = 1LL << (PIL_PREC - 1);
-            for (int k = 0; k < win.n; ++k) acc += (long long)src[(size_t)(win.x0 + k) * d.fw + xs] * pil_tap(win, k);
+            for (int k = 0; k < win.n; ++k) acc += (long long)src[(size_t)(win.x0 + k) * fw + xs] * pil_tap(win, k);
             v = pil_clip8(acc);
         }
-        if constexpr (MODE == REC_SPLIT) return (unsigned short)(v + 1);
-        else return El<MODE == REC_F16 ? 1 : 0>::from_f32(((float)v / 255.0f - 0.5f) / 0.5f);
+        return conv(v);
     };
-    uint16_t* drow = dst + (size_t)y * row_stride;
-    for (int x = imgW + x0; x < imgW + gap; x += 64) drow[x] = 0;
-    int x = x0;
-    for (; x < d.fw; x += 64) drow[x] = sample(x);
-    if (x < imgW) {
-        const uint16_t edge = sample(d.fw - 1);
-        for (; x < imgW; x += 64) drow[x] = edge;
+    bool have_edge = false;
+    uint16_t edge = 0;
+    for (int g = g0; g < ng; g += 1 << lg) {
+        const int c = g * 4;
+        uint16_t v[4];
+        if (c >= imgW) {
+            v[0] = v[1] = v[2] = v[3] = 0;
+        } else if (c + 4 <= fw && !tall && !lut) {
+            uint8_t b[4];
+            __builtin_memcpy(b, src + (size_t)y * rw + c, 4);
+#pragma unroll
+            for (int j = 0; j < 4; ++j) v[j] = conv(b[j]);
+        } else {
+#pragma unroll
+            for (int j = 0; j < 4; ++j) {
+                if (c + j < fw) v[j] = sample(c + j);
+                else if (c + j >= imgW) v[j] = 0;
+                else {
+                    if (!have_edge) { edge = sample(fw - 1); have_edge = true; }
+                    v[j] = edge;
+                }
+            }
+        }
+        const int n = imgW + gap - c;
+        if (wide_ok) {
+            *(uint2*)(drow + c) = make_uint2((unsigned)v[0] | ((unsigned)v[1] << 16), (unsigned)v[2] | ((unsigned)v[3] << 16));
+        } else {
+#pragma unroll
+            for (int j = 0; j < 4; ++j)
+                if (j < n) drow[c + j] = v[j];
+        }
     }
 }
 
@@ -219,11 +285,11 @@
                         int stage_mask, hipStream_t s, int wide_row_stride, int gap, int mode, const CropPage* pages) {
     if (count <= 0) return hipSuccess;
     if ((stage_mask & 1) && pages) {
-        if (any_warp) hipLaunchKernelGGL(crop_warp_kernel<true>, dim3(16, count), dim3(256), 0, s, gray, 0, 0, descs_dev, first, wscratch, pages);
-        hipLaunchKernelGGL(crop_resize_kernel<true>, dim3(16, count), dim3(256), 0, s, gray, 0, 0, descs_dev, first, wscratch, scratch, pages);
+        if (any_warp) hipLaunchKernelGGL(crop_warp_kernel<true>, dim3(CROP_BLOCKS, count), dim3(256), 0, s, gray, 0, 0, descs_dev, first, wscratch, pages);
+        hipLaunchKernelGGL(crop_resize_kernel<true>, dim3(CROP_BLOCKS, count), dim3(256), 0, s, gray, 0, 0, descs_dev, first, wscratch, scratch, pages);
     } else if (stage_mask & 1) {
-        if (any_warp) hipLaunchKernelGGL(crop_warp_kernel<false>, dim3(16, count), dim3(256), 0, s, gray, H, W, descs_dev, first, wscratch, pages);
-        hipLaunchKernelGGL(crop_resize_kernel<false>, dim3(16, count), dim3(256), 0, s, gray, H, W, descs_dev, first, wscratch, scratch, pages);
+        if (any_warp) hipLaunchKernelGGL(crop_warp_kernel<false>, dim3(CROP_BLOCKS, count), dim3(256), 0, s, gray, H, W, descs_dev, first, wscratch, pages);
+        hipLaunchKernelGGL(crop_resize_kernel<false>, dim3(CROP_BLOCKS, count), dim3(256), 0, s, gray, H, W, descs_dev, first, wscratch, scratch, pages);
     }
     if (stage_mask & 2) {
         if (any_tall) hipLaunchKernelGGL(crop_pil_h_kernel, dim3(8, count), dim3(256), 0, s, descs_dev, first, scratch, luts, hscratch);
@@ -231,11 +297,11 @@
         const long long ss = wide_row_stride > 0 ? 1LL : (long long)64 * imgW;
         const int gp = wide_row_stride > 0 ? gap : 0;
         if (mode == REC_SPLIT)
-            hipLaunchKernelGGL(crop_final_kernel<REC_SPLIT>, dim3(16, count), dim3(256), 0, s, descs_dev, first, scratch, hscratch, luts, out_bucket, rs, ss, gp);
+            hipLaunchKernelGGL(crop_final_kernel<REC_SPLIT>, dim3(CROP_BLOCKS, count), dim3(256), 0, s, descs_dev, first, scratch, hscratch, luts, out_bucket, rs, ss, gp);
         else if (mode == REC_F16)
-            hipLaunchKernelGGL(crop_final_kernel<REC_F16>, dim3(16, count), dim3(256), 0, s, descs_dev, first, scratch, hscratch, luts, out_bucket, rs, ss, gp);
+            hipLaunchKernelGGL(crop_final_kernel<REC_F16>, dim3(CROP_BLOCKS, count), dim3(256), 0, s, descs_dev, first, scratch, hscratch, luts, out_bucket, rs, ss, gp);
         else
-            hipLaunchKernelGGL(crop_final_kernel<REC_BF16>, dim3(16, count), dim3(256), 0, s, descs_dev, first, scratch, hscratch, luts, out_bucket, rs, ss, gp);
+            hipLaunchKernelGGL(crop_final_kernel<REC_BF16>, dim3(CROP_BLOCKS, count), dim3(256), 0, s, descs_dev, first, scratch, hscratch, luts, out_bucket, rs, ss, gp);
     }
     return hipGetLastError();
 }
diff --git a/bb-ocr_amd/csrc/ctx.h b/bb-ocr_amd/csrc/ctx.h
--- a/bb-ocr_amd/csrc/ctx.h
+++ b/bb-ocr_amd/csrc/ctx.h
@@ -223,7 +223,7 @@
     DevBuf heat, gray, resized;
     DevBuf pg_rgb, pg_tab;
     PinBuf pg_pin;
-    DevBuf ccl_label, ccl_stat, ccl_slot, ccl_comps, ccl_rowext, ccl_counters;
+    DevBuf ccl_label, ccl_stat, ccl_roots, ccl_comps, ccl_rowext, ccl_counters;
     DevBuf crop_desc, crop_scratch, crop_hscratch, crop_wscratch, crop_luts, crop_hist;
     DevBuf ctc_idx, ctc_pmax, ctc_out_idx, ctc_out, ctc_probs, ctc_beam_idx, ctc_beam_len, ctc_cand, ctc_cand_n, crop_desc2;
     PinBuf desc_pin, desc_pin2;
diff --git a/bb-ocr_amd/csrc/detector.cpp b/bb-ocr_amd/csrc/detector.cpp
--- a/bb-ocr_amd/csrc/detector.cpp
+++ b/bb-ocr_amd/csrc/detector.cpp
@@ -377,7 +377,7 @@
 void ccl_size(bbocr_ctx* c, size_t npx, int cap_comps) {
     c->ccl_label.ensure(npx * 4);
     c->ccl_stat.ensure(npx * 24);
-    c->ccl_slot.ensure(npx * 4);
+    c->ccl_roots.ensure(npx * 4);
     c->ccl_comps.ensure((size_t)cap_comps * sizeof(CclOut));
     c->ccl_rowext.ensure(std::min<size_t>(0x3fffffff, npx) * 8);
     c->ccl_counters.ensure(16);
@@ -393,7 +393,7 @@
     if (!c->ccl_t0) { HIPCHK(hipEventCreate(&c->ccl_t0)); HIPCHK(hipEventCreate(&c->ccl_t1)); }
     HIPCHK(hipEventRecord(c->ccl_t0, st));
     HIPCHK(launch_ccl(heat, B, h, w, (float)p.low_text, (float)p.link_threshold, (double)p.text_threshold, (int*)c->ccl_label.p,
-                      (int*)c->ccl_stat.p, (int*)c->ccl_slot.p, (CclOut*)c->ccl_comps.p, (int*)c->ccl_rowext.p, (int*)c->ccl_counters.p,
+                      (int*)c->ccl_stat.p, (int*)c->ccl_roots.p, (CclOut*)c->ccl_comps.p, (int*)c->ccl_rowext.p, (int*)c->ccl_counters.p,
                       cap_comps, cap_rows, st));
     HIPCHK(hipEventRecord(c->ccl_t1, st));
     int counters[4] = {0, 0, 0, 0};
diff --git a/bb-ocr_amd/csrc/kernels.h b/bb-ocr_amd/csrc/kernels.h
--- a/bb-ocr_amd/csrc/kernels.h
+++ b/bb-ocr_amd/csrc/kernels.h
@@ -113,7 +113,7 @@
     int root, left, top, right, bottom, area, row_off, img;
 };
 hipError_t launch_ccl(const float* heat, int N, int h, int w, float low_text, float link_thr, double text_thr, int* label, int* stat,
-                      int* slot, CclOut* comps, int* rowext, int* counters, int cap_comps, int cap_rows, hipStream_t s);
+                      int* roots, CclOut* comps, int* rowext, int* counters, int cap_comps, int cap_rows, hipStream_t s);
 
 struct CropDesc {
     int img;
```

Result: no change. 970.2 (median of 6 runs) (+0.9%).
